# czbiohub-sf/yogo

Measured on AMD Instinct MI355X. Metric: training images/sec (772x1032 gray), higher is better.
Workload: dtype bf16; 1 GPU; BASELINE configs[2]: full train step (fwd+loss+bwd+clamp+AdamW), base_model, 772x1032x1 uint8, 7 classes; per_gpu_batch=128, global_batch=128, parallelism=dp1

## Files before the change

include/yogo_hip.h:

```cpp
#ifndef YOGO_HIP_H
#define YOGO_HIP_H

#include <stddef.h>

#ifdef __cplusplus
extern "C" {
#endif

typedef void* yogo_stream_t;

const char* yogo_hip_last_error(void);
int yogo_hip_abi_version(void);
int yogo_hip_launch_log(int enable);
int yogo_hip_launch_log_read(char* buf, size_t cap, size_t* needed);


int yogo_conv_packed_bytes(int Cin, int Cout, int ksize, int stride, int mode, size_t* bytes);
int yogo_conv_pack_f32(const float* w_oihw, float* packed, int Cin, int Cout, int ksize, int stride, int mode,
                       yogo_stream_t stream);
int yogo_conv2d_fwd_stats_shape(int B, int Cin, int Cout, int IH, int IW, int ksize, int stride, int* rows, int* mpad);
int yogo_conv2d_fwd_f32(const float* in, const float* packed, const float* bias, float* out, float* out_pre,
                        const float* chan_scale, float* stats_part, int B, int Cin, int Cout, int IH, int IW, int ksize,
                        int stride, int act, yogo_stream_t stream);
int yogo_conv2d_dgrad_f32(const float* dy, const float* packed_dgrad, float* dx, const float* act_ref, int ref_act,
                          const float* chan_scale, int B, int Cin, int Cout, int IH, int IW, int ksize, int stride,
                          yogo_stream_t stream);
int yogo_conv2d_wgrad_workspace_bytes(int B, int Cin, int Cout, int IH, int IW, int ksize, int stride, size_t* bytes);
int yogo_conv2d_wgrad_f32(const float* x, const float* g, float* dw, float* db, void* workspace, int B, int Cin, int Cout,
                          int IH, int IW, int ksize, int stride, float clip, yogo_stream_t stream);

int yogo_conv_first_stats_rows(int B, int IH, int IW, int stride, int* rows);
int yogo_conv_first_fwd(const void* in, int in_dtype, const float* w_oihw, const float* bias, float* out, float* out_pre,
                        const float* chan_scale, float* stats_part, int B, int Cin, int Cout, int IH, int IW, int stride,
                        int act, yogo_stream_t stream);
int yogo_conv_first_wgrad_rows(int B, int IH, int IW, int stride, int* rows);
int yogo_conv_first_wgrad(const void* in, int in_dtype, const float* dy, float* part, int B, int Cin, int Cout, int IH,
                          int IW, int stride, yogo_stream_t stream);

int yogo_bn_finalize(const float* part, int rows, int row_stride, int C, long long count, float eps, float momentum,
                     float* mean_out, float* invstd_out, float* running_mean, float* running_var,
                     long long* num_batches_tracked, yogo_stream_t stream);
int yogo_bn_apply_act(const float* z, float* y, const float* mean, const float* invstd_or_var, int stat_is_var, float eps,
                      const float* gamma, const float* beta, int B, int C, int HW, int act, yogo_stream_t stream);
int yogo_bn_invstd(const float* var, float eps, float* invstd, int C, yogo_stream_t stream);
int yogo_bn_bwd_rows(int B, int HW, int* rows);
int yogo_bn_bwd(const float* g, const float* z, float* dz, const float* mean, const float* invstd, const float* gamma,
                const float* beta, int act, float* dgamma, float* dbeta, float* part, float* sums, int B, int C, int HW,
                int training, float clip, yogo_stream_t stream);
int yogo_partials_reduce(float* part, int rows, int N, float clip, float* out, yogo_stream_t stream);
int yogo_channel_sum(const float* g, int B, int C, int HW, float clip, float* out, yogo_stream_t stream);

int yogo_decode_fwd(const float* raw, float* out, const float* cxs, const float* cys, int B, int P, int Sy, int Sx,
                    float anchor_w, float anchor_h, float width_multiplier, float height_multiplier, int inference,
                    yogo_stream_t stream);
int yogo_decode_bwd(const float* raw, const float* out, const float* gout, float* graw, int B, int P, int Sy, int Sx,
                    int inference, yogo_stream_t stream);

int yogo_decode_bwd_bf16(const float* raw, const float* out, const float* gout, void* graw8c, int B, int P, int Sy, int Sx,
                         int inference, yogo_stream_t stream);

int yogo_loss_workspace_bytes(int B, int Sy, int Sx, size_t* bytes);
int yogo_loss_fwd_bwd(const float* pred, const float* label, float* grad, float* loss_out, void* workspace, int B, int P,
                      int Sy, int Sx, float no_obj_weight, float iou_weight, float classify_weight, float label_smoothing,
                      yogo_stream_t stream);

int yogo_decode_loss_bwd_bf16(const float* raw, const float* label, const float* cxs, const float* cys, void* graw8c, float* loss_out,
                              void* workspace, int B, int P, int Sy, int Sx, float anchor_w, float anchor_h, float width_multiplier,
                              float height_multiplier, float no_obj_weight, float iou_weight, float classify_weight,
                              float label_smoothing, yogo_stream_t stream);

int yogo_format_preds_workspace_bytes(int B, int Sy, int Sx, size_t* bytes);
int yogo_format_preds_batched(const float* pred, float* out_rows, long long* out_cells, int* out_count, void* workspace,
                              int B, int P, int Sy, int Sx, int cap, double obj_thresh, double iou_thresh, int box_format,
                              double min_class_confidence_threshold, yogo_stream_t stream);
int yogo_decode_format_preds_batched(const float* raw, const float* cxs, const float* cys, float* out_rows, long long* out_cells,
                                     int* out_count, void* workspace, int B, int P, int Sy, int Sx, int cap, float anchor_w,
                                     float anchor_h, float width_multiplier, float height_multiplier, int inference,
                                     double obj_thresh, double iou_thresh, int box_format, double min_class_confidence_threshold,
                                     yogo_stream_t stream);
int yogo_head1x1_decode_fwd_bf16(const void* x, const void* packed, const float* bias, float* out, const float* cxs, const float* cys,
                                 int B, int Cin, int P, int Sy, int Sx, float anchor_w, float anchor_h, float width_multiplier,
                                 float height_multiplier, int inference, yogo_stream_t stream);

int yogo_match_workspace_bytes(int B, int Sy, int Sx, int cap, size_t* bytes);
int yogo_match_preds_labels_batched(const float* rows, const int* counts, const float* labels, int* meta, int* pair_label,
                                    int* pair_pred, int* un_label, int* un_pred, float* lab_out, void* workspace, int B, int P, int Sy,
                                    int Sx, int cap, yogo_stream_t stream);
int yogo_match_gather(const float* rows, const float* lab_out, const int* meta, const int* pair_label, const int* pair_pred,
                      const int* un_label, const int* un_pred, float* preds, float* labels, float* missed, float* extra, int B, int P,
                      int cap, long long K, long long Km, long long Ke, yogo_stream_t stream);
int yogo_metrics_state_layout(int C, int T, int nbins, long long* offsets);
int yogo_metrics_accumulate(const float* rows, const float* lab_out, const int* meta, const int* pair_label, const int* pair_pred,
                            const int* un_label, const int* un_pred, const double* roc_thresholds, int T, const double* cal_edges,
                            int nbins, long long* acc, double* bin_conf, double* partial, float* map_rows, long long map_cap, int B,
                            int P, int cap, yogo_stream_t stream);

int yogo_pred_sink_state_layout(int C, long long* offsets);
int yogo_pred_sink_workspace_bytes(int B, size_t* bytes);
int yogo_pred_sink_append(const float* rows, const int* counts, int B, int cap, int P, int mode, int count_classes,
                          long long first_img_id, int img_h, int img_w, long long* state, float* arena, long long arena_cap,
                          int* img_counts, long long img_cap, void* workspace, yogo_stream_t stream);

int yogo_bf16_channel_blocks(int C);
int yogo_conv_bf16_packed_bytes(int Cin, int Cout, int ksize, int mode, size_t* bytes);
int yogo_conv_bf16_pack(const float* w_oihw, const float* scale, void* packed, int Cin, int Cout, int ksize, int mode,
                        yogo_stream_t stream);
int yogo_conv2d_fwd_bf16_stats_shape(int B, int Cin, int Cout, int IH, int IW, int ksize, int stride, int* rows, int* mpad);
int yogo_conv2d_fwd_bf16(const void* in, const void* packed, const float* bias, void* out, float* out_f32,
                         const float* chan_scale, float* stats_part, int B, int Cin, int Cout, int IH, int IW, int ksize,
                         int stride, int act, yogo_stream_t stream);
int yogo_conv2d_fwd_bf16_pre(const void* in, const void* packed, const float* bias, void* out, void* out_pre,
                             const float* chan_scale, int B, int Cin, int Cout, int IH, int IW, int ksize, int stride, int act,
                             yogo_stream_t stream);
int yogo_conv_bf16_pack_blocks(int Cin, int Cout, int ksize, int mode, int* blocks);
int yogo_conv_bf16_pack_multi(const void* table, int n, int total_blocks, yogo_stream_t stream);
int yogo_bf16_signs_bytes(int B, int C, int H, int W, size_t* bytes);
int yogo_conv2d_fwd_bf16_signs(const void* in, const void* packed, const float* bias, void* out, void* signs,
                               const float* chan_scale, int B, int Cin, int Cout, int IH, int IW, int ksize, int stride, int act,
                               yogo_stream_t stream);
int yogo_conv2d_dgrad_bf16_signs(const void* dy, const void* packed_dgrad, void* dx, const void* signs,
                                 const float* chan_scale, int B, int Cin, int Cout, int IH, int IW, int ksize, int stride,
                                 yogo_stream_t stream);
int yogo_conv2d_dgrad_bf16(const void* dy, const void* packed_dgrad, void* dx, const void* act_ref, int ref_act,
                           const float* chan_scale, int B, int Cin, int Cout, int IH, int IW, int ksize, int stride,
                           yogo_stream_t stream);
int yogo_conv2d_wgrad_bf16in(const void* x, const void* g, float* dw, float* db, void* workspace, int B, int Cin, int Cout,
                             int IH, int IW, int ksize, int stride, float clip, yogo_stream_t stream);
int yogo_conv2d_wgrad_bf16_workspace_bytes(int B, int Cin, int Cout, int IH, int IW, int ksize, int stride, size_t* bytes);
int yogo_conv2d_wgrad_bf16(const void* x, const void* g, float* dw, float* db, void* workspace, int B, int Cin, int Cout,
                           int IH, int IW, int ksize, int stride, float clip, yogo_stream_t stream);
int yogo_wgrad_reduce_queue_create(void** queue_out);
int yogo_wgrad_reduce_queue_destroy(void* queue);
int yogo_wgrad_reduce_queue_reset(void* queue);
int yogo_wgrad_reduce_flush(void* queue, yogo_stream_t stream);
int yogo_conv2d_wgrad_bf16_deferred(const void* x, const void* g, float* dw, float* db, void* workspace, int B, int Cin, int Cout, int IH,
                                    int IW, int ks, int stride, float clip, void* queue, yogo_stream_t stream);
int yogo_conv_first_fwd_bf16(const void* in, int in_dtype, const float* w, const float* bias, void* out, int B, int Cin,
                             int Cout, int IH, int IW, int stride, int act, yogo_stream_t stream);
int yogo_conv_first_fwd_train_bf16(const void* in, int in_dtype, const float* w, const float* bias, void* out_bf16,
                                   const float* chan_scale, float* stats_part, int B, int Cin, int Cout, int IH, int IW,
                                   int stride, int act, yogo_stream_t stream);
int yogo_conv_first_wgrad_bf16g(const void* in, int in_dtype, const void* dy_bf16, float* part, int B, int Cin, int Cout,
                                int IH, int IW, int stride, yogo_stream_t stream);
int yogo_conv_first_bn_wgrad_cols(int Cin, int Cout, int* cols);
int yogo_conv_first_bn_wgrad_bf16(const void* in, int in_dtype, const void* g, const void* z, const float* mean,
                                  const float* invstd, const float* gamma, const float* beta, float* part, int B, int Cin,
                                  int Cout, int IH, int IW, int stride, int act, yogo_stream_t stream);
int yogo_conv_first_bn_wgrad_finalize(const float* sums, const float* mean, const float* invstd, const float* gamma,
                                      const float* w_oihw, float* dw, float* dgamma, float* dbeta, int B, int Cin, int Cout,
                                      int IH, int IW, int stride, int training, float clip, yogo_stream_t stream);
int yogo_bn_apply_act_bf16(const void* z, void* y, const float* mean, const float* invstd_or_var, int stat_is_var, float eps,
                           const float* gamma, const float* beta, int B, int C, int HW, int act, yogo_stream_t stream);
int yogo_bn_bwd_bf16_rows(int B, int HW, int* rows);
int yogo_bn_stats_bf16(const void* z, float* part, int B, int C, int HW, yogo_stream_t stream);
int yogo_bn_bwd_bf16(const void* g, const void* z, void* dz, const float* mean, const float* invstd, const float* gamma,
                     const float* beta, int act, float* dgamma, float* dbeta, float* part, float* sums, int B, int C, int HW,
                     int training, float clip, yogo_stream_t stream);
int yogo_bn_bwd_bf16_head(const void* gh, const float* head_w, int P, const void* z, void* dz, const float* mean, const float* invstd,
                          const float* gamma, const float* beta, int act, float* dgamma, float* dbeta, float* part, float* sums, int B,
                          int C, int HW, int training, float clip, yogo_stream_t stream);
int yogo_nchw_f32_to_bf16_8c(const float* in, void* out, int B, int C, int HW, yogo_stream_t stream);
int yogo_bf16_8c_to_nchw_f32(const void* in, float* out, int B, int C, int HW, yogo_stream_t stream);

int yogo_conv_first_mfma_supported(int in_dtype, int Cin, int Cout, int IH, int IW, int stride);
int yogo_conv_first_mfma_stats_rows(int B, int IH, int IW, int* rows);
int yogo_conv_first_mfma(const void* in, const float* w, const float* bias, void* z, void* y, const float* mean,
                         const float* invstd, const float* gamma, const float* beta, float* stats_part, int B, int Cout, int IH,
                         int IW, int act, yogo_stream_t stream);

int yogo_conv_first_gram_rows(int B, int IH, int IW, int* rows);
int yogo_conv_first_gram(const void* in, void* part, double* gram, float* gram_f32, int B, int IH, int IW, yogo_stream_t stream);
int yogo_bn_stats_from_gram(const double* gram, const float* w, const float* bias, int Cout, long long count, float eps,
                            float momentum, float* mean_out, float* invstd_out, float* running_mean, float* running_var,
                            long long* num_batches_tracked, yogo_stream_t stream);
int yogo_conv_first_bn_wgrad_bf16_xg(const void* in, int in_dtype, const void* g, const void* z, const float* mean,
                                     const float* invstd, const float* gamma, const float* beta, float* part, int B, int Cin,
                                     int Cout, int IH, int IW, int stride, int act, yogo_stream_t stream);
int yogo_conv_first_bn_wgrad_finalize_xg(const float* sums, const float* gram, const float* mean, const float* invstd,
                                         const float* gamma, const float* w_oihw, float* dw, float* dgamma, float* dbeta, int B,
                                         int Cin, int Cout, int IH, int IW, int stride, int training, float clip,
                                         yogo_stream_t stream);
int yogo_conv_first_mfma_signs(const void* in, const float* w, const float* bias, void* z, void* y, void* signs, const float* mean,
                               const float* invstd, const float* gamma, const float* beta, int B, int Cout, int IH, int IW, int act,
                               yogo_stream_t stream);
int yogo_conv_first_bn_wgrad_xs_supported(int in_dtype, int Cin, int Cout, int IH, int IW, int stride, int act);
int yogo_conv_first_bn_wgrad_bf16_xs(const void* in, int in_dtype, const void* g, const void* signs, const float* mean,
                                     const float* invstd, const float* gamma, const float* beta, float* part, int B, int Cin,
                                     int Cout, int IH, int IW, int stride, int act, yogo_stream_t stream);
int yogo_conv_first_bn_wgrad_finalize_xs(const float* sums, const float* gram, const float* mean, const float* invstd,
                                         const float* gamma, const float* w_oihw, float* dw, float* dgamma, float* dbeta, int B,
                                         int Cin, int Cout, int IH, int IW, int stride, int training, float clip,
                                         yogo_stream_t stream);
int yogo_conv2d_dgrad_first_bwd_supported(int Cmid, int Cout1, int H, int W, int B, int act0);
int yogo_conv2d_dgrad_first_bwd_rows(int B, int H, int W, int with_wgrad, int* rows);
int yogo_conv2d_dgrad_bf16_first_bwd(const void* g, const void* packed, const void* image, const void* signs, float* part, int B, int Cmid,
                                     int Cout1, int H, int W, int act0, yogo_stream_t stream);
int yogo_conv2d_dgrad_wgrad_first_bwd_workspace_bytes(int B, int H, int W, size_t* bytes);
int yogo_conv2d_dgrad_wgrad_bf16_first_bwd(const void* g, const void* packed, const void* x, const void* image, const void* signs, float* part,
                                           float* dw, float* db, void* workspace, int B, int Cmid, int Cout1, int H, int W, int act0,
                                           float clip, void* queue, yogo_stream_t stream);

int yogo_comm_unique_id_bytes(void);
int yogo_comm_unique_id(void* id_out_host);
int yogo_comm_init(int rank, int world, const void* unique_id_host, void** comm_out);
int yogo_comm_allreduce_flat(void* comm, float* buf, size_t count, yogo_stream_t stream);
int yogo_comm_broadcast_flat(void* comm, void* buf, size_t bytes, int root, yogo_stream_t stream);
int yogo_comm_destroy(void* comm);

int yogo_labels_rasterize(const float* labels, const int* offsets, float* out, int* status, int B, int Sx, int Sy,
                          int box_format, yogo_stream_t stream);
int yogo_flip_batch(const void* img_in, void* img_out, int elem_bytes, const float* lab_in, float* lab_out, int B, int C, int H,
                    int W, int Sy, int Sx, int hflip, int vflip, yogo_stream_t stream);

int yogo_blobgen_max_n(int* n);
int yogo_blobgen_place(const int* table, int num_thumbnails, const int* indices, int S, int n, int H, int W, long long seed,
                       long long epoch, int* boxes, float* rows, int* counts, int* background, yogo_stream_t stream);
int yogo_blobgen_compose(const unsigned char* atlas, long long atlas_bytes, const int* table, const int* boxes, const int* counts,
                         const int* background, const int* positions, int S, int n, int H, int W, void* out, int elem_bytes,
                         yogo_stream_t stream);
int yogo_blobgen_label_rows(const float* rows, const int* counts, int S, int n, float* flat, int* offsets, yogo_stream_t stream);

int yogo_image_cache_gather(const unsigned char* cache, int S, const int* slots, int B, int C, int H, int W, void* out, int out_fp32,
                            yogo_stream_t stream);

int yogo_zarr_unpack(const unsigned char* staged, long long staged_bytes, const long long* tile_off, const int* tile_k, int B, int gh,
                     int gw, int ch, int cw, int cn, int order_f, int fill, int H, int W, int top, int left, int OH, int OW, void* out,
                     int out_fp32, yogo_stream_t stream);

int yogo_adamw_step(float* p, const float* g, float* m, float* v, long long n, int step, double lr, double beta1,
                    double beta2, double eps, double weight_decay, double grad_scale, yogo_stream_t stream);

#ifdef __cplusplus
}
#endif
#endif
```

yogo_amd/csrc/bn.hip:

```cpp
#include "common.h"

__global__ __launch_bounds__(256) void bn_finalize_kernel(const float* __restrict__ part, int rows, int row_stride, int C,
                                                          double count, float eps, float momentum,
                                                          float* __restrict__ mean_out, float* __restrict__ invstd_out,
                                                          float* __restrict__ running_mean, float* __restrict__ running_var,
                                                          long long* __restrict__ num_batches_tracked) {
  __shared__ double sh[2][32][8];
  const int cl = threadIdx.x & 7, slice = threadIdx.x >> 3;
  const int c = blockIdx.x * 8 + cl;
  double s = 0.0, q = 0.0;
  if (c < C) {
    int r = slice;
    for (; r + 7 * 32 < rows; r += 8 * 32) {
      float2 v[8];
#pragma unroll
      for (int j = 0; j < 8; ++j) v[j] = *reinterpret_cast<const float2*>(part + ((size_t)(r + j * 32) * row_stride + c) * 2);
#pragma unroll
      for (int j = 0; j < 8; ++j) {
        s += (double)v[j].x;
        q += (double)v[j].y;
      }
    }
    for (; r < rows; r += 32) {
      const float2 v = *reinterpret_cast<const float2*>(part + ((size_t)r * row_stride + c) * 2);
// ... 211 lines not shown
                       gamma, beta, C, HW, act);
  } else {
    dim3 grid(plane_blocks(HW, 4), B * C);
    hipLaunchKernelGGL((bn_apply_act_kernel<false>), grid, dim3(256), 0, stream, z, y, mean, invstd_or_var, stat_is_var, eps,
                       gamma, beta, C, HW, act);
  }
  YOGO_CHECK_LAUNCH("bn_apply_act");
  return YOGO_OK;
}

extern "C" int yogo_bn_invstd(const float* var, float eps, float* invstd, int C, hipStream_t stream) {
  YOGO_CHECK_ARG(var && invstd && C > 0, "bn_invstd: bad arguments");
  hipLaunchKernelGGL(bn_invstd_kernel, dim3(cdiv(C, 256)), dim3(256), 0, stream, var, eps, invstd, C);
  YOGO_CHECK_LAUNCH("bn_invstd");
  return YOGO_OK;
}

extern "C" int yogo_bn_bwd_rows(int B, int HW, int* rows) {
  YOGO_CHECK_ARG(rows != nullptr, "bn_bwd_rows: null");
  *rows = B * plane_blocks(HW, 8);
  return YOGO_OK;
}

extern "C" int yogo_bn_bwd(const float* g, const float* z, float* dz, const float* mean, const float* invstd,
                           const float* gamma, const float* beta, int act, float* dgamma, float* dbeta, float* part,
                           float* sums, int B, int C, int HW, int training, float clip, hipStream_t stream) {
  YOGO_CHECK_ARG(g && z && dz && mean && invstd && gamma && beta && dgamma && dbeta && part && sums, "bn_bwd: null pointer");
  YOGO_CHECK_ARG(B > 0 && C > 0 && HW > 0, "bn_bwd: bad shape");
  const int nb = plane_blocks(HW, 8);
  hipLaunchKernelGGL(bn_bwd_reduce_kernel, dim3(nb, B * C), dim3(256), 0, stream, g, z, mean, invstd, gamma, beta, act, part, C, HW);
  hipLaunchKernelGGL(bn_bwd_finalize_kernel, dim3(C), dim3(256), 0, stream, part, B * nb, C, clip, dgamma, dbeta, sums, sums + C);
  hipLaunchKernelGGL(bn_bwd_apply_kernel, dim3(nb, B * C), dim3(256), 0, stream, g, z, dz, mean, invstd, gamma, beta, act, sums,
                     sums + C, 1.0f / ((float)B * (float)HW), training, C, HW);
  YOGO_CHECK_LAUNCH("bn_bwd");
  return YOGO_OK;
}

__global__ __launch_bounds__(256) void partials_fold_kernel(float* __restrict__ part, int rows, int N, int S) {
  const int j = blockIdx.x * 256 + threadIdx.x;
  const int s = blockIdx.y;
  if (j >= N) return;
  double acc = 0.0;
  int r = s;
  for (; r + 7 * S < rows; r += 8 * S) {
    float v8[8];
#pragma unroll
    for (int k = 0; k < 8; ++k) v8[k] = part[(size_t)(r + k * S) * N + j];
#pragma unroll
    for (int k = 0; k < 8; ++k) acc += (double)v8[k];
  }
  for (; r < rows; r += S) acc += (double)part[(size_t)r * N + j];
  part[(size_t)s * N + j] = (float)acc;
}

extern "C" int yogo_partials_reduce(float* part, int rows, int N, float clip, float* out, hipStream_t stream) {
  YOGO_CHECK_ARG(part && out && rows > 0 && N > 0, "partials_reduce: bad arguments");
  if (rows > 64) {
    const int S = 64;
    hipLaunchKernelGGL(partials_fold_kernel, dim3(cdiv(N, 256), S), dim3(256), 0, stream, part, rows, N, S);
    rows = S;
  }
  hipLaunchKernelGGL(partials_reduce_kernel, dim3(cdiv(N, 256)), dim3(256), 0, stream, part, rows, N, clip, out);
  YOGO_CHECK_LAUNCH("partials_reduce");
  return YOGO_OK;
}

extern "C" int yogo_channel_sum(const float* g, int B, int C, int HW, float clip, float* out, hipStream_t stream) {
  YOGO_CHECK_ARG(g && out && B > 0 && C > 0 && HW > 0, "channel_sum: bad arguments");
  hipLaunchKernelGGL(channel_sum_kernel, dim3(C), dim3(256), 0, stream, g, B, C, HW, clip, out);
  YOGO_CHECK_LAUNCH("channel_sum");
  return YOGO_OK;
}

typedef __bf16 bf16x8_t __attribute__((ext_vector_type(8)));
typedef unsigned int u32x4_t __attribute__((ext_vector_type(4)));

struct Bn8cParams {
  float mu[8], sc[8], sh[8], ga[8], is[8];
};

__device__ __forceinline__ void bn8c_load(Bn8cParams& q, int cb, int C, const float* mean, const float* invstd_or_var,
                                          int stat_is_var, float eps, const float* gamma, const float* beta) {
#pragma unroll
  for (int j = 0; j < 8; ++j) {
    const int c = min(cb * 8 + j, C - 1);
    const float is = stat_is_var ? 1.0f / sqrtf(invstd_or_var[c] + eps) : invstd_or_var[c];
    q.mu[j] = mean[c];
    q.is[j] = is;
    q.ga[j] = gamma[c];
    q.sc[j] = is * gamma[c];
    q.sh[j] = beta[c];
  }
}

__global__ __launch_bounds__(256) void bn_apply_act_8c_kernel(const u32x4_t* __restrict__ z, u32x4_t* __restrict__ y,
                                                              const float* __restrict__ mean,
                                                              const float* __restrict__ invstd_or_var, int stat_is_var, float eps,
                                                              const float* __restrict__ gamma, const float* __restrict__ beta,
                                                              int C, int Cb, int HW, int act) {
  const int plane = blockIdx.y;
  const int cb = plane % Cb;
  Bn8cParams q;
  bn8c_load(q, cb, C, mean, invstd_or_var, stat_is_var, eps, gamma, beta);
  const u32x4_t* zp = z + (size_t)plane * HW;
  u32x4_t* yp = y + (size_t)plane * HW;
  float sh2[8];
#pragma unroll
  for (int j = 0; j < 8; ++j) sh2[j] = fmaf(-q.mu[j], q.sc[j], q.sh[j]);
  for (int i = blockIdx.x * 256 + threadIdx.x; i < HW; i += gridDim.x * 256) {
    const bf16x8_t v = __builtin_bit_cast(bf16x8_t, zp[i]);
    bf16x8_t o;
#pragma unroll
    for (int j = 0; j < 8; ++j) {
      const float r = act_fwd(fmaf((float)v[j], q.sc[j], sh2[j]), act);
      o[j] = (cb * 8 + j < C) ? (__bf16)r : (__bf16)0.f;
    }
    yp[i] = __builtin_bit_cast(u32x4_t, o);
  }
}

__global__ __launch_bounds__(256) void bn_stats_8c_kernel(const u32x4_t* __restrict__ z, float* __restrict__ part, int C, int Cb,
                                                          int HW) {
  __shared__ float sh[4][16];
  const int plane = blockIdx.y;
  const int cb = plane % Cb, b = plane / Cb;
  const u32x4_t* zp = z + (size_t)plane * HW;
  float s[8], t[8];
#pragma unroll
  for (int j = 0; j < 8; ++j) s[j] = t[j] = 0.f;
  for (int i = blockIdx.x * 256 + threadIdx.x; i < HW; i += gridDim.x * 256) {
    const bf16x8_t zv = __builtin_bit_cast(bf16x8_t, zp[i]);
#pragma unroll
    for (int j = 0; j < 8; ++j) {
      const float v = (float)zv[j];
      s[j] += v;
      t[j] = fmaf(v, v, t[j]);
    }
  }
  const int lane = threadIdx.x & 63, wave = threadIdx.x >> 6;
#pragma unroll
  for (int j = 0; j < 8; ++j) {
    const float a = wave_sum(s[j]), c = wave_sum(t[j]);
    if (lane == 0) {
      sh[wave][2 * j] = a;
      sh[wave][2 * j + 1] = c;
    }
  }
  __syncthreads();
  if (threadIdx.x < 16) {
    const int j = threadIdx.x >> 1;
    if (cb * 8 + j < C)
      part[((size_t)(b * gridDim.x + blockIdx.x) * C + cb * 8 + j) * 2 + (threadIdx.x & 1)] =
          sh[0][threadIdx.x] + sh[1][threadIdx.x] + sh[2][threadIdx.x] + sh[3][threadIdx.x];
  }
}

__global__ __launch_bounds__(256) void bn_bwd_reduce_8c_kernel(const u32x4_t* __restrict__ g, const u32x4_t* __restrict__ z,
                                                               const float* __restrict__ mean, const float* __restrict__ invstd,
                                                               const float* __restrict__ gamma, const float* __restrict__ beta,
                                                               int act, float* __restrict__ part, int C, int Cb, int HW) {
  __shared__ float sh[4][16];
  const int plane = blockIdx.y;
  const int cb = plane % Cb, b = plane / Cb;
  Bn8cParams q;
  bn8c_load(q, cb, C, mean, invstd, 0, 0.f, gamma, beta);
  const u32x4_t* gp = g + (size_t)plane * HW;
  const u32x4_t* zp = z + (size_t)plane * HW;
  float s[8], t[8];
#pragma unroll
  for (int j = 0; j < 8; ++j) s[j] = t[j] = 0.f;
  for (int i = blockIdx.x * 256 + threadIdx.x; i < HW; i += gridDim.x * 256) {
    const bf16x8_t gv = __builtin_bit_cast(bf16x8_t, gp[i]);
    const bf16x8_t zv = __builtin_bit_cast(bf16x8_t, zp[i]);
#pragma unroll
    for (int j = 0; j < 8; ++j) {
      const float xh = ((float)zv[j] - q.mu[j]) * q.is[j];
      const float ge = (float)gv[j] * act_bwd_factor(fmaf(xh, q.ga[j], q.sh[j]), act);
      s[j] += ge;
      t[j] += ge * xh;
    }
  }
  const int lane = threadIdx.x & 63, wave = threadIdx.x >> 6;
#pragma unroll
  for (int j = 0; j < 8; ++j) {
    const float a = wave_sum(s[j]), c = wave_sum(t[j]);
    if (lane == 0) {
      sh[wave][2 * j] = a;
      sh[wave][2 * j + 1] = c;
    }
  }
  __syncthreads();
  if (threadIdx.x < 16) {
    const int j = threadIdx.x >> 1;
    if (cb * 8 + j < C)
      part[((size_t)(b * gridDim.x + blockIdx.x) * C + cb * 8 + j) * 2 + (threadIdx.x & 1)] =
          sh[0][threadIdx.x] + sh[1][threadIdx.x] + sh[2][threadIdx.x] + sh[3][threadIdx.x];
  }
}

__global__ __launch_bounds__(256) void bn_bwd_apply_8c_kernel(const u32x4_t* __restrict__ g, const u32x4_t* __restrict__ z,
                                                              u32x4_t* __restrict__ dz, const float* __restrict__ mean,
                                                              const float* __restrict__ invstd, const float* __restrict__ gamma,
                                                              const float* __restrict__ beta, int act,
                                                              const float* __restrict__ sum_g, const float* __restrict__ sum_gx,
                                                              float inv_count, int training, int C, int Cb, int HW) {
  const int plane = blockIdx.y;
  const int cb = plane % Cb;
  Bn8cParams q;
  bn8c_load(q, cb, C, mean, invstd, 0, 0.f, gamma, beta);
  float mg[8], mgx[8];
#pragma unroll
  for (int j = 0; j < 8; ++j) {
    const int c = min(cb * 8 + j, C - 1);
    mg[j] = training ? sum_g[c] * inv_count : 0.f;
    mgx[j] = training ? sum_gx[c] * inv_count : 0.f;
  }
  const u32x4_t* gp = g + (size_t)plane * HW;
  const u32x4_t* zp = z + (size_t)plane * HW;
  u32x4_t* dp = dz + (size_t)plane * HW;
  for (int i = blockIdx.x * 256 + threadIdx.x; i < HW; i += gridDim.x * 256) {
    const bf16x8_t gv = __builtin_bit_cast(bf16x8_t, gp[i]);
    const bf16x8_t zv = __builtin_bit_cast(bf16x8_t, zp[i]);
    bf16x8_t o;
#pragma unroll
    for (int j = 0; j < 8; ++j) {
      const float xh = ((float)zv[j] - q.mu[j]) * q.is[j];
      const float ge = (float)gv[j] * act_bwd_factor(fmaf(xh, q.ga[j], q.sh[j]), act);
      const float r = q.sc[j] * (ge - mg[j] - xh * mgx[j]);
      o[j] = (cb * 8 + j < C) ? (__bf16)r : (__bf16)0.f;
    }
    dp[i] = __builtin_bit_cast(u32x4_t, o);
  }
}

__global__ __launch_bounds__(256) void nchw_f32_to_8c_kernel(const float* __restrict__ in, u32x4_t* __restrict__ out, int C, int Cb,
                                                             int HW) {
  const int plane = blockIdx.y;
  const int cb = plane % Cb, b = plane / Cb;
  for (int i = blockIdx.x * 256 + threadIdx.x; i < HW; i += gridDim.x * 256) {
    bf16x8_t o;
#pragma unroll
    for (int j = 0; j < 8; ++j) {
      const int c = cb * 8 + j;
      o[j] = (c < C) ? (__bf16)in[((size_t)b * C + c) * HW + i] : (__bf16)0.f;
    }
    out[(size_t)plane * HW + i] = __builtin_bit_cast(u32x4_t, o);
  }
}

__global__ __launch_bounds__(256) void nchw8c_to_f32_kernel(const u32x4_t* __restrict__ in, float* __restrict__ out, int C, int Cb,
                                                            int HW) {
  const int plane = blockIdx.y;
  const int cb = plane % Cb, b = plane / Cb;
  for (int i = blockIdx.x * 256 + threadIdx.x; i < HW; i += gridDim.x * 256) {
    const bf16x8_t v = __builtin_bit_cast(bf16x8_t, in[(size_t)plane * HW + i]);
#pragma unroll
    for (int j = 0; j < 8; ++j) {
      const int c = cb * 8 + j;
      if (c < C) out[((size_t)b * C + c) * HW + i] = (float)v[j];
    }
  }
}

static inline int cb_of(int C) { return ((C + 15) / 16) * 2; }

extern "C" int yogo_bn_apply_act_bf16(const void* z, void* y, const float* mean, const float* invstd_or_var, int stat_is_var,
                                      float eps, const float* gamma, const float* beta, int B, int C, int HW, int act,
                                      hipStream_t stream) {
  YOGO_CHECK_ARG(z && y && mean && invstd_or_var && gamma && beta && C > 0 && HW > 0 && B >= 0, "bn_apply_act_bf16: bad arguments");
  if (B == 0) return YOGO_OK;
  const int Cb = cb_of(C);
  YOGO_CHECK_ARG(B * Cb <= 65535, "bn_apply_act_bf16: batch * channel blocks exceeds 65535");
  hipLaunchKernelGGL(bn_apply_act_8c_kernel, dim3(plane_blocks(HW, 4), B * Cb), dim3(256), 0, stream,
                     reinterpret_cast<const u32x4_t*>(z), reinterpret_cast<u32x4_t*>(y), mean, invstd_or_var, stat_is_var, eps,
                     gamma, beta, C, Cb, HW, act);
  YOGO_CHECK_LAUNCH("bn_apply_act_bf16");
  return YOGO_OK;
}

extern "C" int yogo_bn_bwd_bf16_rows(int B, int HW, int* rows) {
  YOGO_CHECK_ARG(rows != nullptr, "bn_bwd_bf16_rows: null");
  *rows = B * plane_blocks(HW, 4);
  return YOGO_OK;
}

extern "C" int yogo_bn_bwd_bf16(const void* g, const void* z, void* dz, const float* mean, const float* invstd,
                                const float* gamma, const float* beta, int act, float* dgamma, float* dbeta, float* part,
                                float* sums, int B, int C, int HW, int training, float clip, hipStream_t stream) {
  YOGO_CHECK_ARG(g && z && dz && mean && invstd && gamma && beta && dgamma && dbeta && part && sums, "bn_bwd_bf16: null pointer");
  YOGO_CHECK_ARG(B > 0 && C > 0 && HW > 0, "bn_bwd_bf16: bad shape");
  const int Cb = cb_of(C), nb = plane_blocks(HW, 4);
  YOGO_CHECK_ARG(B * Cb <= 65535, "bn_bwd_bf16: batch * channel blocks exceeds 65535");
  const u32x4_t* g4 = reinterpret_cast<const u32x4_t*>(g);
  const u32x4_t* z4 = reinterpret_cast<const u32x4_t*>(z);
  hipLaunchKernelGGL(bn_bwd_reduce_8c_kernel, dim3(nb, B * Cb), dim3(256), 0, stream, g4, z4, mean, invstd, gamma, beta, act, part, C,
                     Cb, HW);
  hipLaunchKernelGGL(bn_bwd_finalize_kernel, dim3(C), dim3(256), 0, stream, part, B * nb, C, clip, dgamma, dbeta, sums, sums + C);
  hipLaunchKernelGGL(bn_bwd_apply_8c_kernel, dim3(nb, B * Cb), dim3(256), 0, stream, g4, z4, reinterpret_cast<u32x4_t*>(dz), mean,
                     invstd, gamma, beta, act, sums, sums + C, 1.0f / ((float)B * (float)HW), training, C, Cb, HW);
  YOGO_CHECK_LAUNCH("bn_bwd_bf16");
  return YOGO_OK;
}

typedef float f32x4_t __attribute__((ext_vector_type(4)));
typedef unsigned int u32x2_t __attribute__((ext_vector_type(2)));
typedef __bf16 bf16x4_t __attribute__((ext_vector_type(4)));
struct BnHeadLane {
  bf16x8_t wop;
  float mu[4], is[4], ga[4], sh[4], sc[4];
};
__device__ __forceinline__ void bn_head_lane(BnHeadLane& L, const float* __restrict__ hw, int P, int C, int cp, int c16, int g4, const float* mean,
                                             const float* invstd, const float* gamma, const float* beta) {
#pragma unroll
  for (int j = 0; j < 8; ++j) {
    const int k = 8 * g4 + j;
    L.wop[j] = (k < P) ? (__bf16)hw[(size_t)k * C + 16 * cp + c16] : (__bf16)0.f;
  }
#pragma unroll
  for (int i = 0; i < 4; ++i) {
    const int c = 16 * cp + 4 * g4 + i;
    L.mu[i] = mean[c]; L.is[i] = invstd[c]; L.ga[i] = gamma[c]; L.sh[i] = beta[c]; L.sc[i] = invstd[c] * gamma[c];
  }
}
__device__ __forceinline__ void bn_head_fetch(const BnHeadLane& L, const u32x4_t* __restrict__ ghp, const u32x2_t* __restrict__ zp2, int HW, int px, int g4,
                                              float (&gb)[4], float (&zf)[4]) {
  const bool valid = px < HW;
  u32x4_t gop = {0u, 0u, 0u, 0u};
  if (valid && g4 < 2) gop = ghp[(size_t)g4 * HW + px];
  u32x2_t zr = {0u, 0u};
  if (valid) zr = zp2[(size_t)px * 2];
  const f32x4_t d = __builtin_amdgcn_mfma_f32_16x16x32_bf16(L.wop, __builtin_bit_cast(bf16x8_t, gop), f32x4_t{0.f, 0.f, 0.f, 0.f}, 0, 0, 0);
  const bf16x4_t zv = __builtin_bit_cast(bf16x4_t, zr);
#pragma unroll
  for (int i = 0; i < 4; ++i) {
    gb[i] = (float)(__bf16)d[i];
    zf[i] = (float)zv[i];
  }
}
__global__ __launch_bounds__(256) void bn_bwd_reduce_head_kernel(const u32x4_t* __restrict__ gh, const float* __restrict__ hw, int P,
                                                                 const u32x4_t* __restrict__ z, const float* __restrict__ mean,
                                                                 const float* __restrict__ invstd, const float* __restrict__ gamma,
                                                                 const float* __restrict__ beta, int act, float* __restrict__ part, int C, int Cb, int HW) {
  __shared__ float sh[4][32];
  const int cp = blockIdx.y % (Cb / 2), b = blockIdx.y / (Cb / 2);
  const int lane = threadIdx.x & 63, wave = threadIdx.x >> 6, c16 = lane & 15, g4 = lane >> 4;
  BnHeadLane L;
  bn_head_lane(L, hw, P, C, cp, c16, g4, mean, invstd, gamma, beta);
  const u32x4_t* ghp = gh + (size_t)b * 2 * HW;
  const u32x2_t* zp2 = reinterpret_cast<const u32x2_t*>(z + ((size_t)b * Cb + 2 * cp + (g4 >> 1)) * HW) + (g4 & 1);
  float s[4] = {0.f, 0.f, 0.f, 0.f}, t[4] = {0.f, 0.f, 0.f, 0.f};
  for (int px0 = (blockIdx.x * 4 + wave) * 16; px0 < HW; px0 += gridDim.x * 64) {
    float gb[4], zf[4];
    bn_head_fetch(L, ghp, zp2, HW, px0 + c16, g4, gb, zf);
#pragma unroll
    for (int i = 0; i < 4; ++i) {
      const float xh = (zf[i] - L.mu[i]) * L.is[i];
      const float ge = gb[i] * act_bwd_factor(fmaf(xh, L.ga[i], L.sh[i]), act);
      s[i] += ge;
      t[i] += ge * xh;
    }
  }
#pragma unroll
  for (int i = 0; i < 4; ++i) {
    float a = s[i], c = t[i];
#pragma unroll
    for (int o = 8; o > 0; o >>= 1) {
      a += __shfl_xor(a, o, 64);
      c += __shfl_xor(c, o, 64);
    }
    if (c16 == 0) {
      sh[wave][2 * (4 * g4 + i)] = a;
      sh[wave][2 * (4 * g4 + i) + 1] = c;
    }
  }
  __syncthreads();
  if (threadIdx.x < 32)
    part[((size_t)(b * gridDim.x + blockIdx.x) * C + 16 * cp + (threadIdx.x >> 1)) * 2 + (threadIdx.x & 1)] =
        sh[0][threadIdx.x] + sh[1][threadIdx.x] + sh[2][threadIdx.x] + sh[3][threadIdx.x];
}
__global__ __launch_bounds__(256) void bn_bwd_apply_head_kernel(const u32x4_t* __restrict__ gh, const float* __restrict__ hw, int P,
                                                                const u32x4_t* __restrict__ z, u32x4_t* __restrict__ dz, const float* __restrict__ mean,
                                                                const float* __restrict__ invstd, const float* __restrict__ gamma,
                                                                const float* __restrict__ beta, int act, const float* __restrict__ sum_g,
                                                                const float* __restrict__ sum_gx, float inv_count, int training, int C, int Cb, int HW) {
  const int cp = blockIdx.y % (Cb / 2), b = blockIdx.y / (Cb / 2);
  const int lane = threadIdx.x & 63, wave = threadIdx.x >> 6, c16 = lane & 15, g4 = lane >> 4;
  BnHeadLane L;
  bn_head_lane(L, hw, P, C, cp, c16, g4, mean, invstd, gamma, beta);
  float mg[4], mgx[4];
#pragma unroll
  for (int i = 0; i < 4; ++i) {
    const int c = 16 * cp + 4 * g4 + i;
    mg[i] = training ? sum_g[c] * inv_count : 0.f;
    mgx[i] = training ? sum_gx[c] * inv_count : 0.f;
  }
  const u32x4_t* ghp = gh + (size_t)b * 2 * HW;
  const size_t plane_u = ((size_t)b * Cb + 2 * cp + (g4 >> 1)) * HW;
  const u32x2_t* zp2 = reinterpret_cast<const u32x2_t*>(z + plane_u) + (g4 & 1);
  u32x2_t* dp2 = reinterpret_cast<u32x2_t*>(dz + plane_u) + (g4 & 1);
  for (int px0 = (blockIdx.x * 4 + wave) * 16; px0 < HW; px0 += gridDim.x * 64) {
    const int px = px0 + c16;
    float gb[4], zf[4];
    bn_head_fetch(L, ghp, zp2, HW, px, g4, gb, zf);
    bf16x4_t o;
#pragma unroll
    for (int i = 0; i < 4; ++i) {
      const float xh = (zf[i] - L.mu[i]) * L.is[i];
      const float ge = gb[i] * act_bwd_factor(fmaf(xh, L.ga[i], L.sh[i]), act);
      o[i] = (__bf16)(L.sc[i] * (ge - mg[i] - xh * mgx[i]));
    }
    if (px < HW) dp2[(size_t)px * 2] = __builtin_bit_cast(u32x2_t, o);
  }
}
extern "C" int yogo_bn_bwd_bf16_head(const void* gh, const float* head_w, int P, const void* z, void* dz, const float* mean, const float* invstd,
                                     const float* gamma, const float* beta, int act, float* dgamma, float* dbeta, float* part, float* sums,
                                     int B, int C, int HW, int training, float clip, hipStream_t stream) {
  YOGO_CHECK_ARG(gh && head_w && z && dz && mean && invstd && gamma && beta && dgamma && dbeta && part && sums, "bn_bwd_bf16_head: null pointer");
  YOGO_CHECK_ARG(B > 0 && C > 0 && (C % 16) == 0 && HW > 0 && P > 0 && P <= 16, "bn_bwd_bf16_head: bad shape");
  const int Cb = cb_of(C), nb = plane_blocks(HW, 4);
  YOGO_CHECK_ARG(B * Cb <= 65535, "bn_bwd_bf16_head: batch * channel blocks exceeds 65535");
  const u32x4_t* g4 = reinterpret_cast<const u32x4_t*>(gh);
  const u32x4_t* z4 = reinterpret_cast<const u32x4_t*>(z);
  if (yogo_launch_log_enabled()) {
    yogo_launch_log("bn_bwd_reduce_head_kernel | B=%d C=%d HW=%d P=%d act=%d grid=%dx%d", B, C, HW, P, act, nb, B * (Cb / 2));
    yogo_launch_log("bn_bwd_apply_head_kernel | B=%d C=%d HW=%d P=%d act=%d training=%d grid=%dx%d", B, C, HW, P, act, training, nb, B * (Cb / 2));
  }
  hipLaunchKernelGGL(bn_bwd_reduce_head_kernel, dim3(nb, B * (Cb / 2)), dim3(256), 0, stream, g4, head_w, P, z4, mean, invstd, gamma, beta, act, part, C, Cb,
                     HW);
  hipLaunchKernelGGL(bn_bwd_finalize_kernel, dim3(C), dim3(256), 0, stream, part, B * nb, C, clip, dgamma, dbeta, sums, sums + C);
  hipLaunchKernelGGL(bn_bwd_apply_head_kernel, dim3(nb, B * (Cb / 2)), dim3(256), 0, stream, g4, head_w, P, z4, reinterpret_cast<u32x4_t*>(dz), mean, invstd,
                     gamma, beta, act, sums, sums + C, 1.0f / ((float)B * (float)HW), training, C, Cb, HW);
  YOGO_CHECK_LAUNCH("bn_bwd_bf16_head");
  return YOGO_OK;
}

extern "C" int yogo_bn_stats_bf16(const void* z, float* part, int B, int C, int HW, hipStream_t stream) {
  YOGO_CHECK_ARG(z && part && B > 0 && C > 0 && HW > 0, "bn_stats_bf16: bad arguments");
  const int Cb = cb_of(C), nb = plane_blocks(HW, 4);
  YOGO_CHECK_ARG(B * Cb <= 65535, "bn_stats_bf16: batch * channel blocks exceeds 65535");
  hipLaunchKernelGGL(bn_stats_8c_kernel, dim3(nb, B * Cb), dim3(256), 0, stream, reinterpret_cast<const u32x4_t*>(z), part, C, Cb, HW);
  YOGO_CHECK_LAUNCH("bn_stats_bf16");
  return YOGO_OK;
}

extern "C" int yogo_nchw_f32_to_bf16_8c(const float* in, void* out, int B, int C, int HW, hipStream_t stream) {
  YOGO_CHECK_ARG(in && out && B > 0 && C > 0 && HW > 0, "nchw_f32_to_bf16_8c: bad arguments");
  const int Cb = cb_of(C);
  hipLaunchKernelGGL(nchw_f32_to_8c_kernel, dim3(plane_blocks(HW, 2), B * Cb), dim3(256), 0, stream, in,
                     reinterpret_cast<u32x4_t*>(out), C, Cb, HW);
  YOGO_CHECK_LAUNCH("nchw_f32_to_bf16_8c");
  return YOGO_OK;
}

extern "C" int yogo_bf16_8c_to_nchw_f32(const void* in, float* out, int B, int C, int HW, hipStream_t stream) {
  YOGO_CHECK_ARG(in && out && B > 0 && C > 0 && HW > 0, "bf16_8c_to_nchw_f32: bad arguments");
  const int Cb = cb_of(C);
  hipLaunchKernelGGL(nchw8c_to_f32_kernel, dim3(plane_blocks(HW, 2), B * Cb), dim3(256), 0, stream,
                     reinterpret_cast<const u32x4_t*>(in), out, C, Cb, HW);
  YOGO_CHECK_LAUNCH("bf16_8c_to_nchw_f32");
  return YOGO_OK;
}
```

yogo_amd/csrc/conv_bf16.hip:

```cpp
#include "common.h"
#include "conv_bf16_ws.h"
#include "conv_bf16_ws16.h"
#include "conv_bf16_ws3.h"
#include <type_traits>
#include <utility>
#include <cstdlib>
#include <vector>

typedef float f32x16 __attribute__((ext_vector_type(16)));
typedef __bf16 bf16x8 __attribute__((ext_vector_type(8)));
typedef __bf16 bf16x4 __attribute__((ext_vector_type(4)));
typedef unsigned int u32x4 __attribute__((ext_vector_type(4)));
typedef unsigned int u32x2 __attribute__((ext_vector_type(2)));
typedef int i32x16 __attribute__((ext_vector_type(16)));

#define BF_MAX_TAPS 9
#define BF_LDS_BUDGET (80 * 1024)
#define BF_LDS_MAX (160 * 1024)

struct ConvBf16Params {
  const u32x4* in;
  const u32x4* wp;
  const float* bias;
  u32x2* out;
// ... 1180 lines not shown
  g_diag_stamps = reinterpret_cast<unsigned long long*>(stamps); g_diag_stamps_bytes = stamps_bytes;
  return YOGO_OK;
}
#endif

namespace {

template <int MW, int NW, int NWV, bool S2D, int PF, bool F32, int REF, bool PP, bool LEPI = false>
void bf_launch_one(dim3 grid, int lds_bytes, hipStream_t stream, const ConvBf16Params& p, const char* plan_txt) {
  static bool attr_set = false;
  if (!attr_set) {
    (void)hipFuncSetAttribute(reinterpret_cast<const void*>(&conv_bf16_kernel<MW, NW, NWV, S2D, PF, F32, REF, PP, LEPI>),
                              hipFuncAttributeMaxDynamicSharedMemorySize, BF_LDS_MAX);
    attr_set = true;
  }
  hipLaunchKernelGGL((conv_bf16_kernel<MW, NW, NWV, S2D, PF, F32, REF, PP, LEPI>), grid, dim3(64 * NWV), lds_bytes, stream, p);
  yogo_launch_log("conv_bf16_kernel<%d, %d, %d, %s, %d, %s, %d, %s, %s> | %s", MW, NW, NWV, S2D ? "true" : "false", PF, F32 ? "true" : "false", REF,
                  PP ? "true" : "false", LEPI ? "true" : "false", plan_txt);
}
template <int MW, int NW, int NWV, bool S2D, int PF, bool F32, int REF>
void bf_launch_t(dim3 grid, int lds_bytes, hipStream_t stream, const ConvBf16Params& p, bool use_pp, const char* plan_txt) {
  if constexpr (NWV == 8 && !S2D && !F32) {
    if (use_pp) {
      bf_launch_one<MW, NW, NWV, S2D, PF, F32, REF, true>(grid, lds_bytes, stream, p, plan_txt);
      return;
    }
  }
  if constexpr (NWV == 4 && !S2D && !F32) {
    if (p.lean4) {
      const bool general = p.stats_part != nullptr || p.act == ACT_SILU || p.out_pre != nullptr || ((REF == 1 || REF == 2) && p.ref_act != ACT_LEAKY);
#ifndef BF_NO_LEPI
      if constexpr (REF != 1) {
        if (!general) {
          bf_launch_one<MW, NW, NWV, S2D, PF, F32, REF, true, true>(grid, lds_bytes, stream, p, plan_txt);
          return;
        }
      }
#else
      (void)general;
#endif
      bf_launch_one<MW, NW, NWV, S2D, PF, F32, REF, true>(grid, lds_bytes, stream, p, plan_txt);
      return;
    }
  }
  if constexpr (NWV == 4 && S2D && !F32 && REF != 1) {
    const bool general = p.stats_part != nullptr || p.act == ACT_SILU || p.out_pre != nullptr || (REF == 2 && p.ref_act != ACT_LEAKY);
    if (!general) {
      bf_launch_one<MW, NW, NWV, S2D, PF, F32, REF, false, true>(grid, lds_bytes, stream, p, plan_txt);
      return;
    }
  }
  bf_launch_one<MW, NW, NWV, S2D, PF, F32, REF, false>(grid, lds_bytes, stream, p, plan_txt);
}

int launch_conv_bf16(const void* in, const void* packed, const float* bias, void* out, float* out_f32, void* out_pre, const void* act_ref,
                     int ref_act, void* signs, bool signs_read, const float* chan_scale, float* stats_part, int B, int K, int M, int IH, int IW, int OH,
                     int OW, int ks, int a, int s2d, int act, hipStream_t stream, int* stats_rows, int* stats_mpad) {
  const int T = ks * ks, pad = ks == 3 ? 1 : 0;
  if (in != nullptr && g_bf_ws && !s2d && a == 1 && ks == 3 && out_f32 == nullptr && out_pre == nullptr && act_ref == nullptr && !signs_read &&
      stats_part == nullptr && (act == ACT_NONE || act == ACT_LEAKY) && !(signs != nullptr && act != ACT_LEAKY) &&
      conv_bf16_ws_eligible(K, M, IH, IW, B)) {
    ConvWsParams q{};
    q.in = in; q.wp = packed; q.bias = bias; q.out = out; q.signs = reinterpret_cast<unsigned char*>(signs); q.chan_scale = chan_scale;
    q.B = B; q.Kb = bf_kb_of(K); q.IH = IH; q.IW = IW; q.act = act;
#ifdef YOGO_DIAG
    q.dbg = g_diag_dbg;
    q.stamps = (g_diag_stamps != nullptr && g_diag_stamps_bytes >= 512 * 128) ? g_diag_stamps : nullptr;
    if (q.stamps) (void)hipMemsetAsync(g_diag_stamps, 0, 512 * 128, stream);
#endif
    if (conv_bf16_ws_plan(&q)) {
      if ((g_bf_ws16 == 2 || (g_bf_ws16 == 1 && bias == nullptr)) && act == ACT_NONE && signs == nullptr && chan_scale == nullptr &&
          conv_bf16_ws16_eligible(K, M, IH, IW, B))
        return launch_conv_bf16_ws16(q, stream);
      return launch_conv_bf16_ws(q, stream);
    }
  }
  if (in != nullptr && g_bf_ws && !s2d && a == 2 && ks == 3 && out_f32 == nullptr && out_pre == nullptr && act_ref == nullptr && !signs_read &&
      stats_part == nullptr && (act == ACT_NONE || act == ACT_LEAKY) && !(signs != nullptr && act != ACT_LEAKY) && conv_bf16_ws3_eligible(K, M, IH, IW, B)) {
    ConvWs3Params q{};
    q.in = in; q.wp = packed; q.bias = bias; q.out = out; q.signs = reinterpret_cast<unsigned char*>(signs); q.chan_scale = chan_scale;
    q.B = B; q.Kb = bf_kb_of(K); q.IH = IH; q.IW = IW; q.OH = OH; q.OW = OW; q.act = act;
#ifdef YOGO_DIAG
    q.dbg = g_diag_dbg;
    q.stamps = (g_diag_stamps != nullptr && g_diag_stamps_bytes >= 512 * 128) ? g_diag_stamps : nullptr;
    if (q.stamps) (void)hipMemsetAsync(g_diag_stamps, 0, 512 * 128, stream);
#endif
    if (conv_bf16_ws3_plan(&q)) return launch_conv_bf16_ws3(q, stream);
  }
  if (in != nullptr && g_bf_head && ks == 1 && a == 1 && !s2d && out_pre == nullptr && act_ref == nullptr && stats_part == nullptr && act == ACT_NONE &&
      out_f32 != nullptr && out == nullptr && signs == nullptr && chan_scale == nullptr && conv_bf16_head_fwd_eligible(K, M, OH * OW, B))
    return launch_conv_bf16_head_fwd(in, packed, bias, out_f32, B, K, M, OH * OW, stream);
  if (in != nullptr && g_bf_staged && !s2d && ks == 3 && out_f32 == nullptr && out_pre == nullptr && act_ref == nullptr && !signs_read && stats_part == nullptr &&
      (act == ACT_NONE || act == ACT_LEAKY) && !(signs != nullptr && act != ACT_LEAKY) && conv_bf16_staged_eligible(K, M, a, IH, IW, OH, OW, B))
    return launch_conv_bf16_staged(in, packed, bias, out, signs, chan_scale, B, K, M, IH, IW, OH, OW, a, act, stream);
  if (in != nullptr && g_bf_direct && s2d && ks == 3 && out_f32 == nullptr && out_pre == nullptr && act_ref == nullptr && bias == nullptr &&
      stats_part == nullptr && act == ACT_NONE && (!signs_read || (signs != nullptr && ref_act == ACT_LEAKY)) && (signs_read || signs == nullptr) &&
      conv_bf16_s2d_direct_eligible(K, M, OH, OW, B))
    return launch_conv_bf16_s2d_direct(in, packed, out, signs_read ? signs : nullptr, chan_scale, B, K, M, IH, IW, OH, OW, stream);
  const int MW = bf_pick_mw(M);
  const bool small_n = s2d || a == 2;
  const bool wide64 = MW == 2 && !small_n && K >= 64 && OH * OW >= 4096;
  const int NW = MW == 1 ? (small_n ? 2 : 4) : (small_n ? 1 : (wide64 ? 4 : 2));
  const int NWV = (MW == 4 || wide64) ? 8 : 4;
  const int PF = NWV == 8 ? 10 : 16;
  const int Kb = bf_kb_of(K), Mpad = bf_mpad_of(M);
  const int OHt = s2d ? (OH + 1) / 2 : OH, OWt = s2d ? (OW + 1) / 2 : OW;
  BfTiling tl;
  bool planned = false;
  if (NWV == 4) {
    const int ladder[3] = {40 * 1024, 53 * 1024, BF_LDS_BUDGET};
    for (int i = 0; i < 3 && !planned; ++i)
      planned = bf_plan(OHt, OWt, s2d ? 1 : a, s2d ? 6 : T, s2d ? 2 : ks, Kb, MW, NW, NWV, PF, ladder[i], &tl) && tl.dma;
  }
  bool ring = false;
  if (s2d && MW == 4 && Kb >= 8 && g_bf_ring) {
    ring = bf_plan(OHt, OWt, 1, 6, 2, Kb, MW, NW, NWV, 5, BF_LDS_MAX, &tl, false, 2, 4, 2);
    planned = ring;
  }
  if (!planned) planned = bf_plan(OHt, OWt, s2d ? 1 : a, s2d ? 6 : T, s2d ? 2 : ks, Kb, MW, NW, NWV, PF, BF_LDS_MAX, &tl);
  if (!planned) {
    yogo_set_error("conv_bf16: no LDS tiling fits (K=%d M=%d OW=%d a=%d)", K, M, OW, a);
    return YOGO_ERR_ARG;
  }
  int rowdma = 0, lwp = 0;
  if (!s2d && NWV == 4 && T == 9 && tl.CKb == 2 && tl.dma == 2 && out_f32 == nullptr && g_bf_lean4 && g_bf_rowdma) {
    const int ladder[3] = {40 * 1024, 53 * 1024, BF_LDS_BUDGET};
    int level = 0;
    while (level < 2 && tl.lds_bytes > ladder[level]) ++level;
    BfTiling tr;
    if (tl.lds_bytes <= ladder[level] && bf_plan_rows(OHt, OWt, a, T, ks, Kb, MW, NW, NWV, ladder[level], &tr, &lwp)) {
      tl = tr;
      rowdma = 1;
    }
  }
  dim3 grid(tl.ncb * tl.tiles_per_band, (Mpad / (32 * MW)) * (s2d ? 2 : 1), B);
  if (stats_rows) *stats_rows = B * (int)grid.x;
  if (stats_mpad) *stats_mpad = Mpad;
  if (in == nullptr) return YOGO_OK;
  ConvBf16Params p{};
  p.in = reinterpret_cast<const u32x4*>(in); p.wp = reinterpret_cast<const u32x4*>(packed); p.bias = bias;
  p.out = reinterpret_cast<u32x2*>(out); p.out_f32 = out_f32; p.out_pre = reinterpret_cast<u32x2*>(out_pre);
  p.act_ref = reinterpret_cast<const u32x2*>(act_ref); p.ref_act = ref_act; p.signs = reinterpret_cast<unsigned char*>(signs); p.chan_scale = chan_scale; p.stats_part = stats_part;
  p.B = B; p.Kb = Kb; p.M = M; p.Mpad = Mpad; p.Mb = bf_kb_of(M);
  p.IH = IH; p.IW = IW; p.OH = OH; p.OW = OW; p.T = T;
  if (s2d) {
    p.a = 1; p.dy_min = 0; p.dx_min = 0; p.span_y = 2; p.span_x = 2;
  } else {
    p.a = a; p.dy_min = -pad; p.dx_min = -pad; p.span_y = ks; p.span_x = ks;
  }
  p.ncb = tl.ncb; p.TW = tl.TW; p.tiles_per_band = tl.tiles_per_band;
  {
    auto magic = [](int d) -> unsigned { return d <= 1 ? 0xFFFFFFFFu : (unsigned)(((1ull << 32) + (unsigned)d - 1ull) / (unsigned)d); };
    const int a_ = s2d ? 1 : a, span_ = s2d ? 2 : ks;
    const int bw_last = OWt - (tl.ncb - 1) * tl.TW;
    p.m_gx = magic((int)grid.x); p.m_gy = magic((int)grid.y); p.m_gxy = magic((int)(grid.x * grid.y)); p.m_tpb = magic(tl.tiles_per_band);
    p.m_bw = magic(tl.TW); p.m_bwl = magic(bw_last);
    p.m_lw = magic((tl.TW - 1) * a_ + span_); p.m_lwl = magic((bw_last - 1) * a_ + span_);
  }
  p.CKb = tl.CKb; p.ckb_shift = tl.CKb == 8 ? 3 : (tl.CKb == 4 ? 2 : 1); p.nchunk = Kb / tl.CKb;
  p.ldsw_off = tl.ldsw_off; p.lds_dummy = tl.lds_dummy; p.act = act;
  p.dma = tl.dma; p.ni_slots = tl.ni_slots; p.n_slots = tl.n_slots; p.bufu = tl.bufu; p.bufs = tl.dma == 1 ? tl.bufu : 0;
  p.ring = ring ? 1 : 0;
  p.lean4 = (!s2d && NWV == 4 && T == 9 && tl.CKb == 2 && tl.dma == 2 && out_f32 == nullptr && g_bf_lean4) ? 1 : 0;
  p.rowdma = rowdma; p.lwp = lwp;
#ifdef YOGO_DIAG
  p.dbg = g_diag_dbg;
  if (g_diag_nodma && (tl.lds_dummy + 1) * 16 <= BF_LDS_MAX) p.dma = 0;
  {
    const size_t nwg = (size_t)grid.x * grid.y * grid.z;
    if (g_diag_stamps != nullptr && nwg * 128 <= g_diag_stamps_bytes) {
      (void)hipMemsetAsync(g_diag_stamps, 0, nwg * 128, stream);
      p.stamps = g_diag_stamps;
    }
  }
#endif
  if ((act_ref != nullptr || signs_read) && bias != nullptr) {
    yogo_set_error("conv_bf16: an activation reference goes with a data gradient (no bias)");
    return YOGO_ERR_ARG;
  }
  if (B == 0) return YOGO_OK;
  int lds_bytes = max(p.dma ? tl.lds_bytes : (tl.lds_dummy + 1) * 16, (2 + 2 * NWV) * 32 * MW * 4);
  const bool use_pp = NWV == 8 && !s2d && T == 9 && p.dma == 1 && tl.CKb == 2 && tl.ni_slots <= 5 && tl.n_slots - tl.ni_slots <= 5 && g_bf_pp;
  if (use_pp) {
    p.ni_slots = 5; p.n_slots = 10; p.ldsw_off = 5 * 64 * NWV; p.bufu = 10 * 64 * NWV; p.bufs = p.bufu;
    lds_bytes = 2 * p.bufu * 16;
  }
  char plan_txt[256] = "";
  if (yogo_launch_log_enabled())
    snprintf(plan_txt, sizeof(plan_txt), "K=%d M=%d in=%dx%d out=%dx%d a=%d s2d=%d T=%d ncb=%d TW=%d tiles_per_band=%d CKb=%d nchunk=%d rows=%d LW=%d lds=%d dma=%d slots=%d+%d rowpitch=%d grid=%ux%ux%u",
             K, M, IH, IW, OH, OW, a, s2d, T, tl.ncb, tl.TW, tl.tiles_per_band, tl.CKb, Kb / tl.CKb, tl.rows_max, tl.LW, lds_bytes, p.dma, tl.ni_slots,
             tl.n_slots - tl.ni_slots, rowdma ? lwp : 0, grid.x, grid.y, grid.z);
#define BFLAUNCH__(MW_, NW_, NWV_, S2D_, PF_, F32_, REF_)                                                               \
  bf_launch_t<MW_, NW_, NWV_, S2D_, PF_, F32_, REF_>(grid, lds_bytes, stream, p, use_pp, plan_txt)
#define BFLAUNCH_(MW_, NW_, NWV_, S2D_, PF_, F32_)                             \
  do {                                                                         \
    if (act_ref != nullptr) BFLAUNCH__(MW_, NW_, NWV_, S2D_, PF_, false, 1);   \
    else if (signs_read) BFLAUNCH__(MW_, NW_, NWV_, S2D_, PF_, false, 2);      \
    else if (signs != nullptr && NWV_ != 8) BFLAUNCH__(MW_, NW_, NWV_, S2D_, PF_, false, 3); \
    else BFLAUNCH__(MW_, NW_, NWV_, S2D_, PF_, F32_, 0);                       \
  } while (0)
#define BFLAUNCH(MW_, NW_, NWV_, S2D_, PF_)                                    \
  do {                                                                         \
    if (out_f32 != nullptr) BFLAUNCH_(MW_, NW_, NWV_, S2D_, PF_, true);        \
    else BFLAUNCH_(MW_, NW_, NWV_, S2D_, PF_, false);                          \
  } while (0)
  if (s2d) {
    if (MW == 4) BFLAUNCH_(4, 1, 8, true, 10, false);
    else if (MW == 2) BFLAUNCH_(2, 1, 4, true, 16, false);
    else BFLAUNCH_(1, 2, 4, true, 16, false);
  } else if (a == 2) {
    if (MW == 4) BFLAUNCH(4, 1, 8, false, 10);
    else if (MW == 2) BFLAUNCH(2, 1, 4, false, 16);
    else BFLAUNCH(1, 2, 4, false, 16);
  } else {
    if (MW == 4) BFLAUNCH(4, 2, 8, false, 10);
    else if (MW == 2 && wide64) BFLAUNCH(2, 4, 8, false, 10);
    else if (MW == 2) BFLAUNCH(2, 2, 4, false, 16);
    else BFLAUNCH(1, 4, 4, false, 16);
  }
#undef BFLAUNCH
#undef BFLAUNCH_
#undef BFLAUNCH__
  YOGO_CHECK_LAUNCH("conv_bf16");
  return YOGO_OK;
}

int check_bf16_conv(int B, int Cin, int Cout, int IH, int IW, int ks, int stride) {
  YOGO_CHECK_ARG((ks == 3 || ks == 1) && (stride == 1 || stride == 2) && !(ks == 1 && stride != 1) && B >= 0 && Cin > 0 &&
                     Cout > 0 && IH > 0 && IW > 0, "conv_bf16: unsupported shape");
  return YOGO_OK;
}

}

extern "C" int yogo_conv2d_fwd_bf16_stats_shape(int B, int Cin, int Cout, int IH, int IW, int ks, int stride, int* rows, int* mpad) {
  if (int e = check_bf16_conv(B, Cin, Cout, IH, IW, ks, stride)) return e;
  const int pad = ks == 3 ? 1 : 0;
  return launch_conv_bf16(nullptr, nullptr, nullptr, nullptr, nullptr, nullptr, nullptr, 0, nullptr, false, nullptr, nullptr, B, Cin, Cout, IH, IW,
                          (IH + 2 * pad - ks) / stride + 1, (IW + 2 * pad - ks) / stride + 1, ks, stride, 0, 0, nullptr, rows, mpad);
}

extern "C" int yogo_conv2d_fwd_bf16(const void* in, const void* packed, const float* bias, void* out, float* out_f32,
                                    const float* chan_scale, float* stats_part, int B, int Cin, int Cout, int IH, int IW,
                                    int ks, int stride, int act, hipStream_t stream) {
  YOGO_CHECK_ARG(in && packed && (out || out_f32), "conv2d_fwd_bf16: null pointer");
  if (int e = check_bf16_conv(B, Cin, Cout, IH, IW, ks, stride)) return e;
  const int pad = ks == 3 ? 1 : 0;
  return launch_conv_bf16(in, packed, bias, out, out_f32, nullptr, nullptr, 0, nullptr, false, chan_scale, stats_part, B, Cin, Cout, IH, IW,
                          (IH + 2 * pad - ks) / stride + 1, (IW + 2 * pad - ks) / stride + 1, ks, stride, 0, act, stream,
                          nullptr, nullptr);
}

extern "C" int yogo_conv2d_fwd_bf16_pre(const void* in, const void* packed, const float* bias, void* out, void* out_pre,
                                        const float* chan_scale, int B, int Cin, int Cout, int IH, int IW, int ks, int stride,
                                        int act, hipStream_t stream) {
  YOGO_CHECK_ARG(in && packed && out && out_pre, "conv2d_fwd_bf16_pre: null pointer");
  if (int e = check_bf16_conv(B, Cin, Cout, IH, IW, ks, stride)) return e;
  const int pad = ks == 3 ? 1 : 0;
  return launch_conv_bf16(in, packed, bias, out, nullptr, out_pre, nullptr, 0, nullptr, false, chan_scale, nullptr, B, Cin, Cout, IH, IW,
                          (IH + 2 * pad - ks) / stride + 1, (IW + 2 * pad - ks) / stride + 1, ks, stride, 0, act, stream,
                          nullptr, nullptr);
}

extern "C" int yogo_bf16_signs_bytes(int B, int C, int H, int W, size_t* bytes) {
  YOGO_CHECK_ARG(bytes && B >= 0 && C > 0 && H > 0 && W > 0, "bf16_signs_bytes: bad arguments");
  *bytes = (size_t)B * H * W * (bf_mpad_of(C) / 8);
  return YOGO_OK;
}

extern "C" int yogo_conv2d_fwd_bf16_signs(const void* in, const void* packed, const float* bias, void* out, void* signs,
                                          const float* chan_scale, int B, int Cin, int Cout, int IH, int IW, int ks, int stride,
                                          int act, hipStream_t stream) {
  YOGO_CHECK_ARG(in && packed && out && signs, "conv2d_fwd_bf16_signs: null pointer");
  if (int e = check_bf16_conv(B, Cin, Cout, IH, IW, ks, stride)) return e;
  const int pad = ks == 3 ? 1 : 0;
  return launch_conv_bf16(in, packed, bias, out, nullptr, nullptr, nullptr, 0, signs, false, chan_scale, nullptr, B, Cin, Cout, IH, IW,
                          (IH + 2 * pad - ks) / stride + 1, (IW + 2 * pad - ks) / stride + 1, ks, stride, 0, act, stream,
                          nullptr, nullptr);
}

extern "C" int yogo_conv2d_dgrad_bf16_signs(const void* dy, const void* packed_dgrad, void* dx, const void* signs,
                                            const float* chan_scale, int B, int Cin, int Cout, int IH, int IW, int ks, int stride,
                                            hipStream_t stream) {
  YOGO_CHECK_ARG(dy && packed_dgrad && dx && signs, "conv2d_dgrad_bf16_signs: null pointer");
  if (int e = check_bf16_conv(B, Cin, Cout, IH, IW, ks, stride)) return e;
  const int pad = ks == 3 ? 1 : 0;
  const int OHf = (IH + 2 * pad - ks) / stride + 1, OWf = (IW + 2 * pad - ks) / stride + 1;
  return launch_conv_bf16(dy, packed_dgrad, nullptr, dx, nullptr, nullptr, nullptr, ACT_LEAKY, const_cast<void*>(signs), true, chan_scale,
                          nullptr, B, Cout, Cin, OHf, OWf, IH, IW, ks, 1, (stride == 2 && ks == 3) ? 1 : 0, ACT_NONE, stream, nullptr,
                          nullptr);
}

extern "C" int yogo_conv2d_dgrad_bf16(const void* dy, const void* packed_dgrad, void* dx, const void* act_ref, int ref_act,
                                      const float* chan_scale, int B, int Cin, int Cout, int IH, int IW, int ks, int stride,
                                      hipStream_t stream) {
  YOGO_CHECK_ARG(dy && packed_dgrad && dx, "conv2d_dgrad_bf16: null pointer");
  if (int e = check_bf16_conv(B, Cin, Cout, IH, IW, ks, stride)) return e;
  const int pad = ks == 3 ? 1 : 0;
  const int OHf = (IH + 2 * pad - ks) / stride + 1, OWf = (IW + 2 * pad - ks) / stride + 1;
  return launch_conv_bf16(dy, packed_dgrad, nullptr, dx, nullptr, nullptr, act_ref, ref_act, nullptr, false, chan_scale, nullptr, B, Cout, Cin, OHf, OWf,
                          IH, IW, ks, 1, (stride == 2 && ks == 3) ? 1 : 0, ACT_NONE, stream, nullptr, nullptr);
}

extern "C" int yogo_conv_first_fwd_bf16(const void* in, int in_dtype, const float* w, const float* bias, void* out, int B,
                                        int Cin, int Cout, int IH, int IW, int stride, int act, hipStream_t stream) {
  YOGO_CHECK_ARG(in && w && out, "conv_first_fwd_bf16: null pointer");
  YOGO_CHECK_ARG((Cin == 1 || Cin == 3) && Cout > 0 && (stride == 1 || stride == 2) && (in_dtype == 0 || in_dtype == 1) && B >= 0,
                 "conv_first_fwd_bf16: unsupported shape");
  ConvFirstBf16Params p{};
  p.in = in; p.w = w; p.bias = bias; p.out = reinterpret_cast<u32x4*>(out);
  p.B = B; p.Cin = Cin; p.Cout = Cout; p.Mb = bf_kb_of(Cout); p.IH = IH; p.IW = IW; p.stride = stride; p.act = act;
  p.OH = (IH - 1) / stride + 1; p.OW = (IW - 1) / stride + 1;
  if (B == 0) return YOGO_OK;
  dim3 grid(cdiv(p.OH * p.OW, 256), B);
  if (in_dtype == 0 && Cin == 1) hipLaunchKernelGGL((conv_first_bf16_kernel<uint8_t, 1>), grid, dim3(256), 0, stream, p);
  else if (in_dtype == 0) hipLaunchKernelGGL((conv_first_bf16_kernel<uint8_t, 3>), grid, dim3(256), 0, stream, p);
  else if (Cin == 1) hipLaunchKernelGGL((conv_first_bf16_kernel<float, 1>), grid, dim3(256), 0, stream, p);
  else hipLaunchKernelGGL((conv_first_bf16_kernel<float, 3>), grid, dim3(256), 0, stream, p);
  YOGO_CHECK_LAUNCH("conv_first_fwd_bf16");
  return YOGO_OK;
}
```

yogo_amd/csrc/conv_bf16_ws.h:

```cpp
#pragma once
#include "common.h"

#define WS_PT 256
#define WS_NT 256
#define WS_NI 4
#define WS_WB (9 * 2 * 128 * 16)
#define WS_IB (WS_NI * WS_NT * 16)
#define WS_I0 (2 * WS_WB)
#define WS_STG (WS_I0 + 3 * WS_IB)
#define WS_EB (WS_STG + 32768)
#define WS_ES (WS_EB + 512)
#define WS_MB (WS_ES + 1024)
#define WS_MBS (WS_MB + 4096)
#define WS_LDS_BYTES (WS_MBS + 16)

struct ConvWsParams {
  const void* in;
  const void* wp;
  const float* bias;
  void* out;
  unsigned char* signs;
  const float* chan_scale;
  int B, Kb, IH, IW;
  int ncb, TW, tiles_per_band, gx, ntiles;
  unsigned m_gx, m_tpb, m_bw, m_bwl, m_lw, m_lwl;
  int nchunk, act;
#ifdef YOGO_DIAG
  int dbg;
  unsigned long long* stamps;
#endif
};

bool conv_bf16_ws_eligible(int K, int M, int IH, int IW, int B);
bool conv_bf16_ws_plan(ConvWsParams* p, int slots = WS_NI);
int launch_conv_bf16_ws(const ConvWsParams& p, hipStream_t stream);
```

yogo_amd/csrc/conv_bf16_ws16.h:

```cpp
#pragma once
#include "conv_bf16_ws.h"

#define W16_WSLOT (3 * 2 * 2 * 128 * 16)
#define W16_W0 0
#define W16_ISLOT (2 * WS_IB)
#define W16_I0 (2 * W16_WSLOT)
#define W16_STG (W16_I0 + 2 * W16_ISLOT)
#define W16_EB (W16_STG + 32768)
#define W16_MB (W16_EB + 512)
#define W16_MBS (W16_MB + 1024)
#define W16_LDS_BYTES (W16_MBS + 16)

bool conv_bf16_ws16_eligible(int K, int M, int IH, int IW, int B);
int launch_conv_bf16_ws16(const ConvWsParams& p, hipStream_t stream);
```

yogo_amd/csrc/conv_bf16_ws16.hip:

```cpp
#include "conv_bf16_ws16.h"
#ifndef W16_ASM_INC
#define W16_ASM_INC "conv_bf16_ws16_asm.inc"
#endif
#include W16_ASM_INC
#ifndef W16_ABL
#define W16_ABL 0
#endif
#include <mutex>
#include <type_traits>
#include <utility>

typedef unsigned int u32x4 __attribute__((ext_vector_type(4)));
typedef int i32x4 __attribute__((ext_vector_type(4)));

#define W16_CLOBBER \
  "memory", "scc", "s87", "s88", "s89", "s90", "s91", "s92", "s93", "s94", "s95", \
  "v16", "v17", "v18", "v19", "v20", "v21", "v22", "v23", "v24", "v25", "v26", "v27", "v28", "v29", "v30", "v31", "v32", "v33", "v34", "v35", "v36", "v37", "v38", "v39", "v40", "v41", "v42", "v43", "v44", "v45", "v46", "v47", "v48", "v49", "v50", "v51", "v52", "v53", "v54", "v55", "v56", "v57", "v58", "v59", "v60", "v61", "v62", "v63", "v64", "v65", "v66", "v67", "v68", "v69", "v70", "v71", "v72", "v73", "v74", "v75", "v76", "v77", "v78", "v79", "v80", "v81", "v82", "v83", "v84", "v85", "v86", "v87", "v88", "v89", "v90", "v91", "v92", "v93", "v94", "v95", \
  "a0","a1","a2","a3","a4","a5","a6","a7","a8","a9","a10","a11","a12","a13","a14","a15","a16","a17","a18","a19","a20","a21","a22","a23","a24","a25","a26","a27","a28","a29","a30","a31","a32","a33","a34","a35","a36","a37","a38","a39","a40","a41","a42","a43","a44","a45","a46","a47","a48","a49","a50","a51","a52","a53","a54","a55","a56","a57","a58","a59","a60","a61","a62","a63","a64","a65","a66","a67","a68","a69","a70","a71","a72","a73","a74","a75","a76","a77","a78","a79","a80","a81","a82","a83","a84","a85","a86","a87","a88","a89","a90","a91","a92","a93","a94","a95","a96","a97","a98","a99","a100","a101","a102","a103","a104","a105","a106","a107","a108","a109","a110","a111","a112","a113","a114","a115","a116","a117","a118","a119","a120","a121","a122","a123","a124","a125","a126","a127","a128","a129","a130","a131","a132","a133","a134","a135","a136","a137","a138","a139","a140","a141","a142","a143","a144","a145","a146","a147","a148","a149","a150","a151","a152","a153","a154","a155","a156","a157","a158","a159"

namespace {

__device__ __forceinline__ int w16_udivm(int n, unsigned m) { return (int)__umulhi((unsigned)n, m); }
__device__ __forceinline__ int w16_udivm1(int n, int d, unsigned m) { return d == 1 ? n : (int)__umulhi((unsigned)n, m); }
__device__ __forceinline__ int w16_lane() {
  int l;
  asm volatile("v_mbcnt_lo_u32_b32 %0, -1, 0\n\tv_mbcnt_hi_u32_b32 %0, -1, %0" : "=v"(l));
  return l;
}
__device__ __forceinline__ i32x4 w16_rsrc(const void* ptr, unsigned bytes) {
  const unsigned long long a = reinterpret_cast<unsigned long long>(ptr);
  return i32x4{(int)(unsigned)a, (int)((unsigned)(a >> 32) & 0xFFFFu), (int)bytes, 0x00020000};
}
__device__ __forceinline__ void w16_dma4(i32x4 rs, unsigned lds, int v0, int v1, int v2, int v3, unsigned soff) {
  asm volatile(
      "s_mov_b32 m0, %5\n\ts_nop 4\n\tbuffer_load_dwordx4 %0, %4, %6 offen lds\n\t"
      "s_add_u32 m0, m0, 4096\n\ts_nop 0\n\tbuffer_load_dwordx4 %1, %4, %6 offen lds\n\t"
      "s_add_u32 m0, m0, 4096\n\ts_nop 0\n\tbuffer_load_dwordx4 %2, %4, %6 offen lds\n\t"
      "s_add_u32 m0, m0, 4096\n\ts_nop 0\n\tbuffer_load_dwordx4 %3, %4, %6 offen lds"
      ::"v"(v0), "v"(v1), "v"(v2), "v"(v3), "s"(rs), "s"(lds), "s"(soff) : "memory", "scc");
}
__device__ __forceinline__ void w16_dma6(i32x4 rs, unsigned lds, int voff, unsigned soff, unsigned sj, unsigned sk) {
  unsigned so;
#define W16_PJ "s_add_u32 m0, m0, 4096\n\ts_add_u32 %0, %0, %5\n\tbuffer_load_dwordx4 %1, %2, %0 offen lds\n\t"
#define W16_PK "s_add_u32 m0, m0, 4096\n\ts_add_u32 %0, %0, %6\n\tbuffer_load_dwordx4 %1, %2, %0 offen lds\n\t"
  asm volatile("s_mov_b32 m0, %3\n\ts_mov_b32 %0, %4\n\ts_nop 4\n\tbuffer_load_dwordx4 %1, %2, %0 offen lds\n\t" W16_PJ W16_PK W16_PJ W16_PK W16_PJ
               : "=&s"(so)
               : "v"(voff), "s"(rs), "s"(lds), "s"(soff), "s"(sj), "s"(sk)
               : "memory", "scc");
#undef W16_PJ
#undef W16_PK
}
__device__ __forceinline__ void w16_store16(u32x4 data, int voff, i32x4 rs, unsigned soff) {
  asm volatile("s_nop 4\n\tbuffer_store_dwordx4 %0, %1, %2, %3 offen" ::"v"(data), "v"(voff), "s"(rs), "s"(soff) : "memory");
}

}

template <bool BIAS>
__global__ __launch_bounds__(512) __attribute__((amdgpu_waves_per_eu(2, 2), amdgpu_num_vgpr(96))) void conv_bf16_ws16_kernel(const ConvWsParams p) {
  extern __shared__ __attribute__((aligned(16))) u32x4 smem4[];
  constexpr unsigned OOB = 0x80000000u;
  const int tid = threadIdx.x;
  const int wave = __builtin_amdgcn_readfirstlane(tid >> 6);
  const int team = wave >> 2, tw = wave & 3;
  float* ldsf = reinterpret_cast<float*>(smem4);
  unsigned char* lds = reinterpret_cast<unsigned char*>(smem4);

  const int OH = p.IH, OW = p.IW;
  const int plane = OH * OW, plane16 = plane * 16;
  const int npairs = p.nchunk >> 1, nper = 3 * npairs;

  const unsigned NV = (unsigned)p.ntiles, G = gridDim.x, slot = blockIdx.x;
  const unsigned xq = NV >> 3, xr = NV & 7;
  struct TileS { int b, j0, bw, p0, p1, lastband; };
  auto find_tile = [&](unsigned& k, TileS& t) -> bool {
    for (;; ++k) {
      const unsigned lin = slot + k * G;
      if (lin >= NV) return false;
      const unsigned xcd = lin & 7;
      const int widx = (int)((xcd < xr ? xcd * (xq + 1) : xr * (xq + 1) + (xcd - xr) * xq) + (lin >> 3));
      const int b = w16_udivm1(widx, p.gx, p.m_gx);
      const int bx = widx - b * p.gx;
      const int cb = w16_udivm1(bx, p.tiles_per_band, p.m_tpb);
      const int tb = bx - cb * p.tiles_per_band;
      const int j0 = cb * p.TW;
      const int bw = min(p.TW, OW - j0);
      const int NPb = OH * bw;
      const int p0 = tb * WS_PT;
      if (p0 >= NPb) continue;
      t.b = b; t.j0 = j0; t.bw = bw; t.p0 = p0; t.p1 = min(p0 + WS_PT, NPb); t.lastband = cb == p.ncb - 1;
      return true;
    }
  };
  auto pix_geom = [&](const TileS& t, int q, unsigned& pbase, int& vo) {
    const unsigned m_bw = t.lastband ? p.m_bwl : p.m_bw;
    const int bw = t.bw;
    const int i_lo = w16_udivm(t.p0, m_bw);
    const int pp = t.p0 + q;
    const bool pv = pp < t.p1;
    const int pc = pv ? pp : (t.p1 - 1);
    const int i = w16_udivm(pc, m_bw), j = pc - i * bw;
    pbase = (unsigned)((i - i_lo) * (bw + 2) + j) * 16u;
    vo = pv ? (i * OW + t.j0 + j) * 16 : (int)OOB;
  };
  auto tile_pitch = [&](const TileS& t, unsigned& lw16, unsigned& perkb16) {
    const unsigned m_bw = t.lastband ? p.m_bwl : p.m_bw;
    const int i_lo = w16_udivm(t.p0, m_bw), i_hi = w16_udivm(t.p1 - 1, m_bw);
    lw16 = (unsigned)(t.bw + 2) * 16u;
    perkb16 = (unsigned)(i_hi - i_lo + 3) * lw16;
  };

  unsigned k_ord = 0;
  TileS T{};
  if (!find_tile(k_ord, T)) return;

  if (tid < 128) ldsf[W16_EB / 4 + tid] = (BIAS && p.bias != nullptr) ? p.bias[tid] : 0.f;
  __syncthreads();

  if (team == 1) {
    const int lane = w16_lane();
    const int ttid = tw * 64 + lane;
    const int rowb = p.IW * 16, kcb = p.IH * p.IW * 16;
    const unsigned ibytes = (unsigned)p.Kb * kcb, obytes = 16u * plane16, wbytes = 9u * p.Kb * 2048u;
    const unsigned so_i = 2u * kcb;
    const unsigned wstep = (unsigned)p.Kb * 2048u;
    const i32x4 rs_w = w16_rsrc(p.wp, wbytes);
    const int lane16 = lane * 16;
    const int kbw = tw >> 1, colh = tw & 1;
    auto decode_slots = [&](const TileS& t, int (&voff)[WS_NI]) {
      const unsigned m_bw = t.lastband ? p.m_bwl : p.m_bw;
      const int bw = t.bw;
      const int i_lo = w16_udivm(t.p0, m_bw), i_hi = w16_udivm(t.p1 - 1, m_bw);
      const int rows_in = i_hi - i_lo + 3;
      const int iy0 = i_lo - 1, ix0 = t.j0 - 1;
      const int lw = bw + 2;
      const int per_kb = rows_in * lw;
      const unsigned inv_lw = t.lastband ? p.m_lwl : p.m_lw;
      const unsigned inv_perkb = 0xFFFFFFFFu / (unsigned)per_kb + 1u;
      const int skc = w16_udivm(WS_NT, inv_perkb);
      const int srm = WS_NT - skc * per_kb;
      const int sr = w16_udivm(srm, inv_lw);
      const int sx = srm - sr * lw;
      int kc_ = w16_udivm(ttid, inv_perkb);
      const int rm0 = ttid - kc_ * per_kb;
      int r_ = w16_udivm(rm0, inv_lw);
      int x_ = rm0 - r_ * lw;
#pragma unroll
      for (int i = 0; i < WS_NI; ++i) {
        const int iy_ = iy0 + r_, ix_ = ix0 + x_;
        const bool ok = (kc_ < 2) && (iy_ >= 0) && (iy_ < p.IH) && (ix_ >= 0) && (ix_ < p.IW);
        voff[i] = ok ? kc_ * kcb + iy_ * rowb + ix_ * 16 : (int)OOB;
        x_ += sx; r_ += sr; kc_ += skc;
        if (x_ >= lw) { x_ -= lw; ++r_; }
        if (r_ >= rows_in) { r_ -= rows_in; ++kc_; }
      }
    };
    static_assert(WS_NI == 4, "w16_dma4 issues the four input slots");
    auto req_w = [&](int P, int r, int par) {
      const unsigned soff = (unsigned)(((3 * r) * p.Kb + 4 * P + kbw) * 2048 + colh * 1024);
      w16_dma6(rs_w, (unsigned)(W16_W0 + par * W16_WSLOT + kbw * 2048 + colh * 1024), lane16, soff, 4096u, wstep - 4096u);
    };
    auto req_i = [&](i32x4 rs, const int (&voff)[WS_NI], int cn, int ps, int j) {
      w16_dma4(rs, (unsigned)(W16_I0 + ps * W16_ISLOT + j * WS_IB + tw * 64 * 16), voff[0], voff[1], voff[2], voff[3], (unsigned)cn * so_i);
    };
    const unsigned stg_rd = (unsigned)(W16_STG + tw * 8192 + lane * 16);
    u32x4 fifo[8];
    int f_vo = (int)OOB;
    i32x4 f_rs = w16_rsrc(p.out, 0u);
    int f_cb0 = 0;
    auto fifo_fill = [&](int cb0, int vop, i32x4 rs_o) {
#pragma unroll
      for (int u = 0; u < 8; ++u) fifo[u] = *reinterpret_cast<const u32x4*>(lds + stg_rd + u * 1024);
      f_vo = vop; f_rs = rs_o; f_cb0 = cb0;
    };
    auto fifo_store4 = [&](auto h_tag) {
      constexpr int Hh = decltype(h_tag)::value;
      const i32x4 rs = {__builtin_amdgcn_readfirstlane(f_rs.x), __builtin_amdgcn_readfirstlane(f_rs.y), __builtin_amdgcn_readfirstlane(f_rs.z),
                        __builtin_amdgcn_readfirstlane(f_rs.w)};
      const int cb0 = __builtin_amdgcn_readfirstlane(f_cb0);
#pragma unroll
      for (int u = 4 * Hh; u < 4 * Hh + 4; ++u) w16_store16(fifo[u], (W16_ABL & 2) ? (int)OOB : f_vo, rs, (unsigned)(cb0 + u) * (unsigned)plane16);
    };
    using IC0 = std::integral_constant<int, 0>;
    using IC1 = std::integral_constant<int, 1>;

    int voff[WS_NI];
    decode_slots(T, voff);
    unsigned pbase_ = 0, lw16_ = 0, perkb16_ = 0;
    int vo = (int)OOB, vo_prev = (int)OOB;
    pix_geom(T, ttid, pbase_, vo);
    i32x4 rs_in = w16_rsrc(reinterpret_cast<const unsigned char*>(p.in) + (size_t)T.b * ibytes, ibytes);
    i32x4 rs_out = w16_rsrc(reinterpret_cast<unsigned char*>(p.out) + (size_t)T.b * obytes, obytes);
    i32x4 rs_out_prev = w16_rsrc(p.out, 0u);
    req_i(rs_in, voff, 0, 0, 0);
    req_i(rs_in, voff, 1, 0, 1);
    req_w(0, 0, 0);
    asm volatile("s_waitcnt vmcnt(0)" ::: "memory");
    __builtin_amdgcn_s_barrier();
    bool has_next = true;
    TileS Tn{};
    int voff_n[WS_NI] = {(int)OOB, (int)OOB, (int)OOB, (int)OOB}, vo_n = (int)OOB;
    i32x4 rs_in_n = rs_in, rs_out_n = rs_out;
    while (has_next) {
      int P = 0, r = 0;
      for (int c = 0; c < nper; ++c) {
        {
          const int rn = r == 2 ? 0 : r + 1, Pn = r == 2 ? P + 1 : P;
          if ((W16_ABL & 1) && c >= 1) {
          } else if (c + 1 < nper) req_w(Pn, rn, (c + 1) & 1);
          else if (has_next) req_w(0, 0, 0);
        }
        if (c == 0) {
          fifo_fill(0, vo_prev, rs_out_prev);
          asm volatile("s_waitcnt lgkmcnt(0)" ::: "memory");
          if (!(W16_ABL & 4)) __builtin_amdgcn_s_barrier();
        }
        bool req = false;
        if (r < 2 && !(W16_ABL & 8)) {
          if (P + 1 < npairs) {
            req_i(rs_in, voff, 2 * (P + 1) + r, (P + 1) & 1, r);
            req = true;
          } else if (has_next) {
            if (r == 0) {
#pragma unroll
              for (int i = 0; i < WS_NI; ++i) voff[i] = voff_n[i];
              rs_in = rs_in_n;
            }
            req_i(rs_in, voff, r, 0, r);
            req = true;
          }
        }
        if (c == 0) fifo_store4(IC0{});
        else if (c == 1) fifo_store4(IC1{});
        else if (c == 2) { fifo_fill(8, vo_prev, rs_out_prev); fifo_store4(IC0{}); }
        else if (c == 3) fifo_store4(IC1{});
        const bool dr = c < 4;
        if (c == 0) {
          unsigned kn = k_ord + 1;
          has_next = find_tile(kn, Tn);
          k_ord = kn;
          if (has_next) {
            decode_slots(Tn, voff_n);
            pix_geom(Tn, ttid, pbase_, vo_n);
            tile_pitch(Tn, lw16_, perkb16_);
            rs_in_n = w16_rsrc(reinterpret_cast<const unsigned char*>(p.in) + (size_t)Tn.b * ibytes, ibytes);
            rs_out_n = w16_rsrc(reinterpret_cast<unsigned char*>(p.out) + (size_t)Tn.b * obytes, obytes);
          }
        }
        if (c == 1) {
          *reinterpret_cast<unsigned*>(lds + W16_MB + tw * 256 + ((lane & 15) * 4 + (lane >> 4)) * 4) = pbase_;
          if (tw == 0 && lane == 0) *reinterpret_cast<u32x4*>(lds + W16_MBS) = u32x4{has_next ? 1u : 0u, lw16_, perkb16_, 0u};
          asm volatile("s_waitcnt lgkmcnt(0)" ::: "memory");
        }
        if (dr && req) asm volatile("s_waitcnt vmcnt(8)" ::: "memory");
        else if (dr || req) asm volatile("s_waitcnt vmcnt(4)" ::: "memory");
        else asm volatile("s_waitcnt vmcnt(0)" ::: "memory");
        __builtin_amdgcn_s_barrier();
        if (++r == 3) { r = 0; ++P; }
      }
      vo_prev = vo;
      rs_out_prev = rs_out;
      if (has_next) {
        vo = vo_n;
        rs_out = rs_out_n;
      }
    }
    fifo_fill(0, vo_prev, rs_out_prev);
    asm volatile("s_waitcnt lgkmcnt(0)" ::: "memory");
    if (!(W16_ABL & 4)) __builtin_amdgcn_s_barrier();
    fifo_store4(IC0{});
    fifo_store4(IC1{});
    __builtin_amdgcn_s_barrier();
    fifo_fill(8, vo_prev, rs_out_prev);
    fifo_store4(IC0{});
    fifo_store4(IC1{});
    return;
  }

  __builtin_amdgcn_s_setprio(3);
  const int lane = w16_lane(), c16 = lane & 15, g = lane >> 4;
  const unsigned pa_lane = (unsigned)(W16_W0 + (g >> 1) * 4096 + (g & 1) * 2048 + c16 * 16);
  const unsigned stg = (unsigned)(W16_STG + tw * 8192 + (g >> 1) * 1024 + c16 * 16 + (g & 1) * 8);
  const unsigned eb = (unsigned)(W16_EB + g * 16);
  unsigned lw16, perkb16;
  tile_pitch(T, lw16, perkb16);
  unsigned pbl[4];
#pragma unroll
  for (int pb = 0; pb < 4; ++pb) {
    unsigned pbase;
    int vo_unused;
    pix_geom(T, tw * 64 + pb * 16 + c16, pbase, vo_unused);
    pbl[pb] = pbase + (unsigned)(g & 1) * perkb16 + (unsigned)(g >> 1) * (unsigned)WS_IB + (unsigned)W16_I0;
  }
  __builtin_amdgcn_s_barrier();
  const unsigned kmask = (g & 1) ? 0xFFFFFFFFu : 0u, kconst = (unsigned)(g >> 1) * (unsigned)WS_IB + (unsigned)W16_I0;
  const unsigned mba = (unsigned)(W16_MB + tw * 256 + c16 * 16), mbs = (unsigned)W16_MBS;
  const unsigned npp = (unsigned)((nper - 2) >> 1);
  if constexpr (BIAS)
    asm volatile(W16_TXT_ROLEB
                 :
                 : [pa] "v"(pa_lane), [stg] "v"(stg), [eb] "v"(eb), [q0] "v"(pbl[0]), [q1] "v"(pbl[1]), [q2] "v"(pbl[2]), [q3] "v"(pbl[3]), [mba] "v"(mba),
                   [mbs] "v"(mbs), [kmask] "v"(kmask), [kconst] "v"(kconst), [lw16] "s"(lw16), [npp] "s"(npp)
                 : W16_CLOBBER);
  else
    asm volatile(W16_TXT_ROLE
                 :
                 : [pa] "v"(pa_lane), [stg] "v"(stg), [eb] "v"(eb), [q0] "v"(pbl[0]), [q1] "v"(pbl[1]), [q2] "v"(pbl[2]), [q3] "v"(pbl[3]), [mba] "v"(mba),
                   [mbs] "v"(mbs), [kmask] "v"(kmask), [kconst] "v"(kconst), [lw16] "s"(lw16), [npp] "s"(npp)
                 : W16_CLOBBER);
}

bool conv_bf16_ws16_eligible(int K, int M, int IH, int IW, int B) {
  const int Kb = round_up(K, 16) / 8;
  if (!conv_bf16_ws_eligible(K, M, IH, IW, B)) return false;
  return Kb >= 8 && (Kb % 8) == 0;
}

int launch_conv_bf16_ws16(const ConvWsParams& p, hipStream_t stream) {
  static std::mutex mu;
  static int n_cu_of[64] = {0};
  int dev = 0;
  if (hipGetDevice(&dev) != hipSuccess || dev < 0 || dev >= 64) {
    yogo_set_error("conv_bf16_ws16: hipGetDevice failed");
    return YOGO_ERR_HIP;
  }
  int n_cu;
  {
    std::lock_guard<std::mutex> lk(mu);
    if (n_cu_of[dev] == 0) {
      hipError_t e = hipFuncSetAttribute(reinterpret_cast<const void*>(&conv_bf16_ws16_kernel<false>), hipFuncAttributeMaxDynamicSharedMemorySize, W16_LDS_BYTES);
      if (e == hipSuccess)
        e = hipFuncSetAttribute(reinterpret_cast<const void*>(&conv_bf16_ws16_kernel<true>), hipFuncAttributeMaxDynamicSharedMemorySize, W16_LDS_BYTES);
      if (e != hipSuccess) {
        yogo_set_error("conv_bf16_ws16: hipFuncSetAttribute(MaxDynamicSharedMemorySize = %d) failed: %s", W16_LDS_BYTES, hipGetErrorString(e));
        return YOGO_ERR_HIP;
      }
      hipDeviceProp_t prop;
      n_cu_of[dev] = (hipGetDeviceProperties(&prop, dev) == hipSuccess && prop.multiProcessorCount > 0) ? prop.multiProcessorCount : 256;
    }
    n_cu = n_cu_of[dev];
  }
  if (p.ntiles <= 0) return YOGO_OK;
  if (p.act != ACT_NONE || p.signs != nullptr || p.chan_scale != nullptr || (p.nchunk & 3) != 0) {
    yogo_set_error("conv_bf16_ws16: plain epilogue and whole chunk-pair pairs only");
    return YOGO_ERR_ARG;
  }
  int grid = min(p.ntiles, n_cu);
  if (grid >= 8) grid &= ~7;
  if (p.bias != nullptr) hipLaunchKernelGGL(conv_bf16_ws16_kernel<true>, dim3(grid), dim3(512), W16_LDS_BYTES, stream, p);
  else hipLaunchKernelGGL(conv_bf16_ws16_kernel<false>, dim3(grid), dim3(512), W16_LDS_BYTES, stream, p);
  if (yogo_launch_log_enabled())
    yogo_launch_log("conv_bf16_ws16_kernel<%s> | Kb=%d in=%dx%d ncb=%d TW=%d tiles_per_band=%d periods=%d ntiles=%d grid=%d lds=%d", p.bias ? "true" : "false", p.Kb,
                    p.IH, p.IW, p.ncb, p.TW, p.tiles_per_band, 3 * (p.nchunk / 2), p.ntiles, grid, W16_LDS_BYTES);
  YOGO_CHECK_LAUNCH("conv_bf16_ws16");
  return YOGO_OK;
}
```

yogo_amd/engine.py:

```python
from __future__ import annotations

import threading
import weakref
from dataclasses import dataclass, field
from typing import Dict, List, Optional, Tuple

import torch
from torch import nn

from yogo_amd import _hip

ACT_NONE, ACT_LEAKY, ACT_SILU = 0, 1, 2


@dataclass
class Layer:
    conv: nn.Conv2d
    bn: Optional[nn.BatchNorm2d] = None
    act: int = ACT_NONE
    drop: Optional[nn.Dropout2d] = None

    @property
    def cin(self) -> int:
        return self.conv.in_channels
# ... 22 lines not shown
    z: Optional[torch.Tensor] = None
    pre: Optional[torch.Tensor] = None
    signs: Optional[torch.Tensor] = None
    signs0: Optional[torch.Tensor] = None
    w_used: Optional[torch.Tensor] = None
    gram: Optional[torch.Tensor] = None
    mask: Optional[torch.Tensor] = None
    mean: Optional[torch.Tensor] = None
    invstd: Optional[torch.Tensor] = None
    bn_train: bool = False


def parse_backbone(backbone: nn.Sequential) -> List[Layer]:
    layers: List[Layer] = []
    for blk in backbone:
        mods = [blk] if isinstance(blk, nn.Conv2d) else list(blk)
        if not mods or not isinstance(mods[0], nn.Conv2d):
            raise RuntimeError(f"yogo_amd: unsupported block {blk!r}: every block must start with nn.Conv2d")
        conv = mods[0]
        k, s, p = conv.kernel_size, conv.stride, conv.padding
        ok = k[0] == k[1] and s[0] == s[1] and conv.dilation == (1, 1) and conv.groups == 1 and conv.padding_mode == "zeros"
        ok = ok and ((k[0] == 3 and p == (1, 1) and s[0] in (1, 2)) or (k[0] == 1 and p == (0, 0) and s[0] == 1))
        if not ok:
            raise RuntimeError(f"yogo_amd: unsupported convolution {conv!r} (3x3 pad 1 stride 1|2, or 1x1)")
        L = Layer(conv=conv)
        for m in mods[1:]:
            if isinstance(m, nn.BatchNorm2d):
                L.bn = m
            elif isinstance(m, nn.LeakyReLU):
                if abs(m.negative_slope - 0.01) > 1e-12:
                    raise RuntimeError("yogo_amd: LeakyReLU slope must be 0.01")
                L.act = ACT_LEAKY
            elif isinstance(m, nn.SiLU):
                L.act = ACT_SILU
            elif isinstance(m, nn.Dropout2d):
                L.drop = m
            else:
                raise RuntimeError(f"yogo_amd: unsupported module {m!r} in block")
        if L.bn is not None and L.drop is not None:
            raise RuntimeError("yogo_amd: BatchNorm + Dropout2d in one block is not part of the block grammar")
        layers.append(L)
    return layers


def _f32(t: torch.Tensor) -> torch.Tensor:
    return t if (t.dtype == torch.float32 and t.is_contiguous()) else t.contiguous().float()


def _bn_affine(L: Layer, dev) -> Tuple[torch.Tensor, torch.Tensor]:
    bn = L.bn
    gamma = _f32(bn.weight.detach()) if bn.weight is not None else torch.ones(L.cout, device=dev)
    beta = _f32(bn.bias.detach()) if bn.bias is not None else torch.zeros(L.cout, device=dev)
    return gamma, beta


def _bn_grad_dst(bn: nn.BatchNorm2d, dst, grads: Dict[int, torch.Tensor], cout: int, dev) -> Tuple[torch.Tensor, torch.Tensor]:
    dgamma = dst(bn.weight) if bn.weight is not None else torch.empty(cout, dtype=torch.float32, device=dev)
    dbeta = dst(bn.bias) if bn.bias is not None else torch.empty(cout, dtype=torch.float32, device=dev)
    if bn.weight is not None:
        grads[id(bn.weight)] = dgamma
        grads[id(bn.bias)] = dbeta
    return dgamma, dbeta


def _bn_finalize(eng: "Engine", L: Layer, fn: str, *lead_args, count: int, dev, st) -> Tuple[torch.Tensor, torch.Tensor]:
    bn = L.bn
    mean = torch.empty(L.cout, dtype=torch.float32, device=dev)
    invstd = torch.empty(L.cout, dtype=torch.float32, device=dev)
    track = bn.track_running_stats and bn.running_mean is not None
    _hip.call(fn, *lead_args, L.cout, count, float(bn.eps), float(bn.momentum if bn.momentum is not None else 0.0), mean, invstd,
              bn.running_mean if track else None, bn.running_var if track else None, bn.num_batches_tracked if track else None, st)
    if track:
        eng.generation += 1
    return mean, invstd


def _pack_hit(eng: "Engine", key: Tuple[int, int], w: torch.Tensor) -> Optional[torch.Tensor]:
    hit = eng._pack.get(key)
    return hit[2] if hit is not None and hit[0] == w._version and hit[1] == w.data_ptr() else None


class Engine:
    def __init__(self, backbone: nn.Sequential):
        self.backbone_ref = weakref.ref(backbone)
        self.layers = parse_backbone(backbone)
        self._pack: Dict[Tuple[int, int], Tuple[int, int, torch.Tensor]] = {}
        self.clip: float = 0.0
        self.prof: Optional[list] = None
        self.prof_only: Optional[set] = None
        self._open = None
        self.generation: int = 0
        self._pack_multi = None
        self._drop_consts = None
        self._infer_bf16: Optional["InferEngineBF16"] = None

    def _tick(self, kind: str, layer: int, flops: float, mw: int = 0, nbytes: float = 0.0) -> None:
        if self.prof is not None and (self.prof_only is None or mw in self.prof_only):
            e0, e1 = torch.cuda.Event(enable_timing=True), torch.cuda.Event(enable_timing=True)
            e0.record()
            self._open = (kind, layer, mw, flops, e0, e1, nbytes)

    def _tock(self) -> None:
        if self._open is not None:
            self._open[5].record()
            self.prof.append(self._open)
            self._open = None

    def invalidate_packed(self) -> None:
        self._pack.clear()
        self.generation += 1

    def _packed(self, i: int, mode: int) -> torch.Tensor:
        L = self.layers[i]
        w = L.conv.weight
        key = (i, mode)
        buf = _pack_hit(self, key, w)
        if buf is not None:
            return buf
        nbytes = _hip.query_size("yogo_conv_packed_bytes", L.cin, L.cout, L.k, L.s, mode)
        buf = torch.empty(nbytes // 4, dtype=torch.float32, device=w.device)
        _hip.call("yogo_conv_pack_f32", _f32(w.detach()), buf, L.cin, L.cout, L.k, L.s, mode, _hip.stream_ptr())
        self._pack[key] = (w._version, w.data_ptr(), buf)
        return buf

    def _first_direct(self, i: int) -> bool:
        L = self.layers[i]
        return i == 0 and L.cin in (1, 3) and L.k == 3

    def forward(self, x: torch.Tensor, need_grad: bool) -> Tuple[torch.Tensor, List[Saved]]:
        _hip.require_cuda(x, "the input batch")
        if x.ndim != 4:
            raise RuntimeError(f"yogo_amd: expected a [B,C,H,W] batch, got {tuple(x.shape)}")
        dev = x.device
        st = _hip.stream_ptr()
        B = x.shape[0]
        if x.dtype == torch.uint8:
            cur = x.contiguous()
        else:
            cur = _f32(x)
        saved: List[Saved] = []
        for i, L in enumerate(self.layers):
            if cur.shape[1] != L.cin:
                raise RuntimeError(f"yogo_amd: layer {i} expects {L.cin} channels, got {cur.shape[1]}")
            IH, IW = int(cur.shape[2]), int(cur.shape[3])
            OH, OW = L.out_hw(IH, IW)
            if OH <= 0 or OW <= 0:
                raise RuntimeError(f"yogo_amd: image too small at layer {i}")
            w = L.conv.weight
            _hip.require_cuda(w, "the model parameters")
            bias = _f32(L.conv.bias.detach()) if L.conv.bias is not None else None
            S = Saved(x_in=cur)
            mask = None
            if L.drop is not None and L.drop.training and L.drop.p > 0:
                p = float(L.drop.p)
                mask = (torch.rand(B, L.cout, device=dev) >= p).to(torch.float32) / (1.0 - p)
                S.mask = mask
            has_bn = L.bn is not None
            bn_train = has_bn and (L.bn.training or L.bn.running_mean is None)
            out = torch.empty(B, L.cout, OH, OW, dtype=torch.float32, device=dev)
            pre = None
            if (not has_bn) and need_grad and L.act == ACT_SILU:
                pre = torch.empty_like(out)
            stats = None
            rows = mpad = 0
            direct = self._first_direct(i)
            if bn_train:
                if direct:
                    rows = _hip.query_ints("yogo_conv_first_stats_rows", 1, B, IH, IW, L.s)[0]
                    mpad = L.cout
                else:
                    rows, mpad = _hip.query_ints("yogo_conv2d_fwd_stats_shape", 2, B, L.cin, L.cout, IH, IW, L.k, L.s)
                stats = torch.empty(rows * mpad * 2, dtype=torch.float32, device=dev)
            fused_act = ACT_NONE if has_bn else L.act
            if direct:
                _hip.call("yogo_conv_first_fwd", cur, 0 if cur.dtype == torch.uint8 else 1, _f32(w.detach()), bias, out, pre,
                          mask, stats, B, L.cin, L.cout, IH, IW, L.s, fused_act, st)
            else:
                if cur.dtype != torch.float32:
                    cur = cur.float()
                    S.x_in = cur
                pk = self._packed(i, 0)
                self._tick("fwd", i, 2.0 * B * L.cout * L.cin * L.k * L.k * OH * OW, mw=4 if L.cout > 64 else (2 if L.cout > 32 else 1))
                _hip.call("yogo_conv2d_fwd_f32", cur, pk, bias, out, pre, mask, stats, B, L.cin, L.cout, IH, IW, L.k, L.s,
                          fused_act, st)
                self._tock()
            if has_bn:
                bn = L.bn
                gamma, beta = _bn_affine(L, dev)
                y = torch.empty_like(out) if need_grad else out
                if bn_train:
                    if bn.track_running_stats and bn.running_mean is not None and bn.momentum is None:
                        raise RuntimeError("yogo_amd: BatchNorm2d(momentum=None) is not supported")
                    mean, invstd = _bn_finalize(self, L, "yogo_bn_finalize", stats, rows, mpad, count=B * OH * OW, dev=dev, st=st)
                    _hip.call("yogo_bn_apply_act", out, y, mean, invstd, 0, float(bn.eps), gamma, beta, B, L.cout, OH * OW,
                              L.act, st)
                    S.mean, S.invstd = mean, invstd
                else:
                    _hip.call("yogo_bn_apply_act", out, y, bn.running_mean, bn.running_var, 1, float(bn.eps), gamma, beta, B,
                              L.cout, OH * OW, L.act, st)
                    if need_grad:
                        invstd = torch.empty(L.cout, dtype=torch.float32, device=dev)
                        _hip.call("yogo_bn_invstd", bn.running_var, float(bn.eps), invstd, L.cout, st)
                        S.mean, S.invstd = bn.running_mean, invstd
                S.bn_train = bn_train
                S.z = out if need_grad else None
                S.y = y
                cur = y
            else:
                S.y = out
                S.pre = pre
                cur = out
            saved.append(S if need_grad else Saved(x_in=cur))
        return cur, saved

    def backward(self, saved: List[Saved], graw: torch.Tensor,
                 grad_out: Optional[Dict[int, torch.Tensor]] = None, on_layer=None) -> List[Optional[torch.Tensor]]:
        st = _hip.stream_ptr()
        dev = graw.device
        clip = float(self.clip)
        grads: Dict[int, torch.Tensor] = {}

        def dst(param: torch.Tensor) -> torch.Tensor:
            if grad_out is not None and id(param) in grad_out:
                return grad_out[id(param)]
            return torch.empty(param.shape, dtype=torch.float32, device=dev)
        g = _f32(graw)
        n = len(self.layers)
        if g is graw and self.layers[-1].bn is not None:
            g = g.clone()
        for i in range(n - 1, -1, -1):
            L, S = self.layers[i], saved[i]
            B, _, OH, OW = g.shape
            IH, IW = int(S.x_in.shape[2]), int(S.x_in.shape[3])
            if L.bn is not None:
                bn = L.bn
                gamma, beta = _bn_affine(L, dev)
                dgamma, dbeta = _bn_grad_dst(bn, dst, grads, L.cout, dev)
                rows = _hip.query_ints("yogo_bn_bwd_rows", 1, B, OH * OW)[0]
                part = torch.empty(rows * L.cout * 2, dtype=torch.float32, device=dev)
                sums = torch.empty(2 * L.cout, dtype=torch.float32, device=dev)
                _hip.call("yogo_bn_bwd", g, S.z, g, S.mean, S.invstd, gamma, beta, L.act, dgamma, dbeta, part, sums, B, L.cout,
                          OH * OW, 1 if S.bn_train else 0, clip, st)
            dw = dst(L.conv.weight)
            has_bias = L.conv.bias is not None
            if self._first_direct(i):
                rows = _hip.query_ints("yogo_conv_first_wgrad_rows", 1, B, IH, IW, L.s)[0]
                nj = L.cin * 9 + 1
                part = torch.empty(rows * L.cout * nj, dtype=torch.float32, device=dev)
                x_in = S.x_in
                _hip.call("yogo_conv_first_wgrad", x_in, 0 if x_in.dtype == torch.uint8 else 1, g, part, B, L.cin, L.cout, IH,
                          IW, L.s, st)
                red = torch.empty(L.cout, nj, dtype=torch.float32, device=dev)
                _hip.call("yogo_partials_reduce", part, rows, L.cout * nj, clip, red, st)
                dw.copy_(red[:, : nj - 1].reshape(dw.shape))
                if has_bias:
                    db = dst(L.conv.bias)
                    db.copy_(red[:, nj - 1])
                    grads[id(L.conv.bias)] = db
            else:
                wsb = _hip.query_size("yogo_conv2d_wgrad_workspace_bytes", B, L.cin, L.cout, IH, IW, L.k, L.s)
                ws = torch.empty(wsb // 4, dtype=torch.float32, device=dev)
                db = dst(L.conv.bias) if has_bias else None
                self._tick("wgrad", i, 2.0 * B * L.cout * L.cin * L.k * L.k * OH * OW)
                _hip.call("yogo_conv2d_wgrad_f32", S.x_in, g, dw, db, ws, B, L.cin, L.cout, IH, IW, L.k, L.s, clip, st)
                self._tock()
                if has_bias:
                    grads[id(L.conv.bias)] = db
            grads[id(L.conv.weight)] = dw
            if on_layer is not None:
                on_layer(i)
            if i > 0:
                Lp, Sp = self.layers[i - 1], saved[i - 1]
                ref_act = Lp.act
                if Lp.bn is not None:
                    act_ref, ref_act = None, ACT_NONE
                elif Lp.act == ACT_SILU:
                    act_ref = Sp.pre
                    if act_ref is None:
                        raise RuntimeError("yogo_amd: missing saved pre-activation for a SiLU block")
                elif Lp.act == ACT_LEAKY:
                    act_ref = Sp.y
                else:
                    act_ref = None
                dx = torch.empty(B, L.cin, IH, IW, dtype=torch.float32, device=dev)
                pk = self._packed(i, 1)
                mw_tag = 20 if L.s == 2 else (4 if L.cin > 64 else (2 if L.cin > 32 else 1))
                self._tick("dgrad", i, 2.0 * B * L.cout * L.cin * L.k * L.k * OH * OW, mw=mw_tag)
                _hip.call("yogo_conv2d_dgrad_f32", g, pk, dx, act_ref, ref_act, Sp.mask, B, L.cin, L.cout, IH, IW, L.k, L.s, st)
                self._tock()
                g = dx
        bb = self.backbone_ref()
        return [grads.get(id(p)) for p in bb.parameters()]



def _blocks(c: int) -> int:
    return ((c + 15) // 16) * 2


_FUSE_LAYER0_BWD = True
_L0_NO_Z = True
_WGRAD_DEFER_REDUCE = True
_L01_FUSE_BWD = True
_HEAD_BN_FUSE = True


def _packed_bf16(eng: Engine, i: int, mode: int) -> torch.Tensor:
    L = eng.layers[i]
    w = L.conv.weight
    key = (i, 10 + mode)
    buf = _pack_hit(eng, key, w)
    if buf is not None:
        return buf
    nbytes = _hip.query_size("yogo_conv_bf16_packed_bytes", L.cin, L.cout, L.k, mode)
    buf = torch.empty(nbytes, dtype=torch.uint8, device=w.device)
    _hip.call("yogo_conv_bf16_pack", _f32(w.detach()), None, buf, L.cin, L.cout, L.k, mode, _hip.stream_ptr())
    eng._pack[key] = (w._version, w.data_ptr(), buf)
    return buf


def _pack_all_bf16(eng: Engine) -> None:
    jobs = [(i, mode) for i in range(1, len(eng.layers)) for mode in (0, 2 if (eng.layers[i].s == 2 and eng.layers[i].k == 3) else 1)]
    ws = [eng.layers[i].conv.weight for i, _ in jobs]
    if any(w.dtype != torch.float32 or not w.is_contiguous() for w in ws) or not jobs:
        return
    if all(_pack_hit(eng, (i, 10 + m), w) is not None for (i, m), w in zip(jobs, ws)):
        return
    dev = ws[0].device
    key = tuple(w.data_ptr() for w in ws)
    st = eng._pack_multi
    if st is None or st[0] != key:
        bufs, rows, blk = [], [], 0
        for (i, mode), w in zip(jobs, ws):
            L = eng.layers[i]
            buf = torch.empty(_hip.query_size("yogo_conv_bf16_packed_bytes", L.cin, L.cout, L.k, mode), dtype=torch.uint8, device=dev)
            bufs.append(buf)
            rows.append([w.data_ptr(), 0, buf.data_ptr(), L.cin, L.cout, L.k, mode, blk])
            blk += _hip.query_ints("yogo_conv_bf16_pack_blocks", 1, L.cin, L.cout, L.k, mode)[0]
        st = (key, bufs, torch.tensor(rows, dtype=torch.int64, device=dev), blk)
        eng._pack_multi = st
    _, bufs, table, blk = st
    _hip.call("yogo_conv_bf16_pack_multi", table, len(jobs), blk, _hip.stream_ptr())
    for (i, mode), w, buf in zip(jobs, ws, bufs):
        eng._pack[(i, 10 + mode)] = (w._version, w.data_ptr(), buf)


def _dropout_masks(eng: Engine, B: int, dev) -> Dict[int, torch.Tensor]:
    act = [(i, float(L.drop.p)) for i, L in enumerate(eng.layers) if L.drop is not None and L.drop.training and L.drop.p > 0]
    if not act:
        return {}
    key = (B, tuple(act), str(dev))
    cached = eng._drop_consts
    if cached is None or cached[0] != key:
        sizes = [B * eng.layers[i].cout for i, _ in act]
        pvec = torch.cat([torch.full((n,), p, dtype=torch.float32) for n, (_, p) in zip(sizes, act)]).to(dev)
        cached = (key, sizes, pvec, 1.0 / (1.0 - pvec))
        eng._drop_consts = cached
    _, sizes, pvec, inv_keep = cached
    m = (torch.rand(pvec.numel(), device=dev) >= pvec).to(torch.float32) * inv_keep
    out, off = {}, 0
    for n, (i, _) in zip(sizes, act):
        out[i] = m[off:off + n].view(B, eng.layers[i].cout)
        off += n
    return out


def _check_bf16_train_input(eng: Engine, x: torch.Tensor) -> None:
    _hip.require_cuda(x, "the input batch")
    if x.ndim != 4:
        raise RuntimeError(f"yogo_amd: expected a [B,C,H,W] batch, got {tuple(x.shape)}")
    if x.shape[1] != eng.layers[0].cin:
        raise RuntimeError(f"yogo_amd: layer 0 expects {eng.layers[0].cin} channels, got {x.shape[1]}")
    for j in range(1, len(eng.layers)):
        if eng.layers[j].cin != eng.layers[j - 1].cout:
            raise RuntimeError(f"yogo_amd: layer {j} expects {eng.layers[j].cin} channels, layer {j - 1} produces {eng.layers[j - 1].cout}")
    for Lj in eng.layers:
        bnj = Lj.bn
        if (bnj is not None and (bnj.training or bnj.running_mean is None) and bnj.track_running_stats
                and bnj.running_mean is not None and bnj.momentum is None):
            raise RuntimeError("yogo_amd: BatchNorm2d(momentum=None) is not supported")
    if not eng._first_direct(0):
        raise RuntimeError("yogo_amd: bf16 training needs a 1- or 3-channel 3x3 first convolution")


def _first_mfma_fwd_bf16(eng: Engine, L: Layer, S: Saved, bias, bn_train: bool, B: int, H: int, W: int, st) -> torch.Tensor:
    cur, dev = S.x_in, S.x_in.device
    OH, OW = L.out_hw(H, W)
    bn = L.bn
    gamma, beta = _bn_affine(L, dev)
    w32 = _f32(L.conv.weight.detach())
    y = torch.empty(B, _blocks(L.cout), OH, OW, 8, dtype=torch.bfloat16, device=dev)
    if bn_train:
        rows = _hip.query_ints("yogo_conv_first_gram_rows", 1, B, H, W)[0]
        gpart = torch.empty(rows * 54, dtype=torch.int32, device=dev)
        gram64 = torch.empty(90, dtype=torch.float64, device=dev)
        S.gram = torch.empty(90, dtype=torch.float32, device=dev)
        _hip.call("yogo_conv_first_gram", cur, gpart, gram64, S.gram, B, H, W, st)
        mean, invstd = _bn_finalize(eng, L, "yogo_bn_stats_from_gram", gram64, w32, bias, count=B * OH * OW, dev=dev, st=st)
    else:
        invstd = torch.empty(L.cout, dtype=torch.float32, device=dev)
        _hip.call("yogo_bn_invstd", bn.running_var, float(bn.eps), invstd, L.cout, st)
        mean = bn.running_mean
    no_z = (_L0_NO_Z and _FUSE_LAYER0_BWD and S.gram is not None and L.conv.bias is None
            and _hip.lib().yogo_conv_first_bn_wgrad_xs_supported(0, L.cin, L.cout, H, W, L.s, L.act))
    if no_z:
        out8 = None
        S.signs0 = torch.empty(B, OH * OW * 2, dtype=torch.uint8, device=dev)
        _hip.call("yogo_conv_first_mfma_signs", cur, w32, bias, None, y, S.signs0, mean, invstd, gamma, beta, B, L.cout, H, W, L.act, st)
    else:
        out8 = torch.empty_like(y)
        _hip.call("yogo_conv_first_mfma", cur, w32, bias, out8, y, mean, invstd, gamma, beta, None, B, L.cout, H, W, L.act, st)
    S.mean, S.invstd, S.bn_train, S.z, S.y = mean, invstd, bn_train, out8, y
    S.w_used = w32.to(torch.bfloat16).to(torch.float32)
    return y


def _layer_fwd_bf16(eng: Engine, i: int, L: Layer, S: Saved, bias, bn_train: bool, last: bool, B: int, H: int, W: int, st) -> torch.Tensor:
    cur, mask, dev = S.x_in, S.mask, S.x_in.device
    OH, OW = L.out_hw(H, W)
    has_bn = L.bn is not None
    if last and (has_bn or mask is not None):
        raise RuntimeError("yogo_amd: BatchNorm / Dropout on the last layer is not supported by the bf16 path")
    fused_act = ACT_NONE if has_bn else L.act
    out8 = None if last else torch.empty(B, _blocks(L.cout), OH, OW, 8, dtype=torch.bfloat16, device=dev)
    out32 = torch.empty(B, L.cout, OH, OW, dtype=torch.float32, device=dev) if last else None
    stats = None
    rows = mpad = 0
    if i == 0:
        if bn_train:
            rows, mpad = _hip.query_ints("yogo_conv_first_stats_rows", 1, B, H, W, L.s)[0], L.cout
            stats = torch.empty(rows * mpad * 2, dtype=torch.float32, device=dev)
        _hip.call("yogo_conv_first_fwd_train_bf16", cur, 0 if cur.dtype == torch.uint8 else 1, _f32(L.conv.weight.detach()), bias,
                  out8, mask, stats, B, L.cin, L.cout, H, W, L.s, fused_act, st)
    else:
        pk = _packed_bf16(eng, i, 0)
        nbytes = B * (_blocks(L.cin) * 8 * H * W * 2 + (L.cout * OH * OW * 4 if last else _blocks(L.cout) * 8 * OH * OW * 2))
        eng._tick("fwd", i, 2.0 * B * L.cout * L.cin * L.k * L.k * OH * OW, mw=34 if (L.cout > 64 and L.s == 1) else (35 if (L.cout > 64 and L.cin > 64 and L.k == 3) else 30), nbytes=nbytes)
        if L.act == ACT_SILU and not has_bn:
            S.pre = torch.empty_like(out8)
            _hip.call("yogo_conv2d_fwd_bf16_pre", cur, pk, bias, out8, S.pre, mask, B, L.cin, L.cout, H, W, L.k, L.s, fused_act, st)
        elif L.act == ACT_LEAKY and not has_bn and not last:
            S.signs = torch.empty(_hip.query_size("yogo_bf16_signs_bytes", B, L.cout, OH, OW), dtype=torch.uint8, device=dev)
            _hip.call("yogo_conv2d_fwd_bf16_signs", cur, pk, bias, out8, S.signs, mask, B, L.cin, L.cout, H, W, L.k, L.s, fused_act, st)
        else:
            _hip.call("yogo_conv2d_fwd_bf16", cur, pk, bias, out8, out32, mask, None, B, L.cin, L.cout, H, W, L.k, L.s, fused_act, st)
        eng._tock()
    if not has_bn:
        S.y = out32 if last else out8
        return S.y
    bn = L.bn
    gamma, beta = _bn_affine(L, dev)
    y = torch.empty_like(out8)
    if bn_train:
        if i > 0:
            rows, mpad = _hip.query_ints("yogo_bn_bwd_bf16_rows", 1, B, OH * OW)[0], L.cout
            stats = torch.empty(rows * mpad * 2, dtype=torch.float32, device=dev)
            _hip.call("yogo_bn_stats_bf16", out8, stats, B, L.cout, OH * OW, st)
        mean, invstd = _bn_finalize(eng, L, "yogo_bn_finalize", stats, rows, mpad, count=B * OH * OW, dev=dev, st=st)
    else:
        invstd = torch.empty(L.cout, dtype=torch.float32, device=dev)
        _hip.call("yogo_bn_invstd", bn.running_var, float(bn.eps), invstd, L.cout, st)
        mean = bn.running_mean
    _hip.call("yogo_bn_apply_act_bf16", out8, y, mean, invstd, 0, float(bn.eps), gamma, beta, B, L.cout, OH * OW, L.act, st)
    S.mean, S.invstd, S.bn_train, S.z, S.y = mean, invstd, bn_train, out8, y
    return y


def forward_bf16_train(eng: Engine, x: torch.Tensor) -> Tuple[torch.Tensor, List[Saved]]:
    _check_bf16_train_input(eng, x)
    dev, st, B = x.device, _hip.stream_ptr(), x.shape[0]
    _pack_all_bf16(eng)
    masks = _dropout_masks(eng, B, dev)
    cur = x.contiguous() if x.dtype == torch.uint8 else _f32(x)
    H, W = int(cur.shape[2]), int(cur.shape[3])
    saved: List[Saved] = []
    n = len(eng.layers)
    for i, L in enumerate(eng.layers):
        OH, OW = L.out_hw(H, W)
        if OH <= 0 or OW <= 0:
            raise RuntimeError(f"yogo_amd: image too small at layer {i}")
        last = i == n - 1
        has_bn = L.bn is not None
        if L.act == ACT_SILU and not has_bn and (i == 0 or last):
            raise RuntimeError("yogo_amd: bf16 training of a first / last SiLU block without BatchNorm is not implemented (use fp32)")
        bias = _f32(L.conv.bias.detach()) if L.conv.bias is not None else None
        S = Saved(x_in=cur, mask=masks.get(i))
        bn_train = has_bn and (L.bn.training or L.bn.running_mean is None)
        if (i == 0 and has_bn and S.mask is None and not last and cur.dtype == torch.uint8
                and _hip.lib().yogo_conv_first_mfma_supported(0, L.cin, L.cout, H, W, L.s)):
            cur = _first_mfma_fwd_bf16(eng, L, S, bias, bn_train, B, H, W, st)
        else:
            cur = _layer_fwd_bf16(eng, i, L, S, bias, bn_train, last, B, H, W, st)
        saved.append(S)
        H, W = OH, OW
    return cur, saved


def backward_bf16_train(eng: Engine, saved: List[Saved], graw: torch.Tensor,
                        grad_out: Optional[Dict[int, torch.Tensor]] = None, on_layer=None,
                        trace: Optional[dict] = None, flush_layers=None, stop_at: int = 0) -> List[Optional[torch.Tensor]]:
    n = len(eng.layers)
    if not 0 <= stop_at < n:
        raise ValueError(f"yogo_amd: stop_at {stop_at} is not a layer of this {n}-layer network")
    st, dev, clip = _hip.stream_ptr(), graw.device, float(eng.clip)
    grads: Dict[int, torch.Tensor] = {}

    def dst(param: torch.Tensor) -> torch.Tensor:
        if grad_out is not None and id(param) in grad_out:
            return grad_out[id(param)]
        return torch.empty(param.shape, dtype=torch.float32, device=dev)

    queued_ws: List[torch.Tensor] = []
    wq = _wgrad_queue() if (_WGRAD_DEFER_REDUCE and (on_layer is None or flush_layers is not None)) else None
    flush_at = frozenset(flush_layers) if flush_layers is not None else frozenset()
    if wq is not None:
        _hip.call("yogo_wgrad_reduce_queue_reset", wq)
    if graw.dtype == torch.bfloat16 and graw.ndim == 5:
        g = graw
        B = g.shape[0]
    else:
        graw = _f32(graw)
        B, P, Sy, Sx = graw.shape
        g = torch.empty(B, _blocks(P), Sy, Sx, 8, dtype=torch.bfloat16, device=dev)
        _hip.call("yogo_nchw_f32_to_bf16_8c", graw, g, B, P, Sy * Sx, st)

    def bn_backward(L, S, g, head_g, OH, OW):
        gamma, beta = _bn_affine(L, dev)
        dgamma, dbeta = _bn_grad_dst(L.bn, dst, grads, L.cout, dev)
        rows = _hip.query_ints("yogo_bn_bwd_bf16_rows", 1, B, OH * OW)[0]
        part = torch.empty(rows * L.cout * 2, dtype=torch.float32, device=dev)
        sums = torch.empty(2 * L.cout, dtype=torch.float32, device=dev)
        if head_g is not None:
            dz = torch.empty(B, _blocks(L.cout), OH, OW, 8, dtype=torch.bfloat16, device=dev)
            _hip.call("yogo_bn_bwd_bf16_head", *head_g, S.z, dz, S.mean, S.invstd, gamma, beta, L.act, dgamma, dbeta,
                      part, sums, B, L.cout, OH * OW, 1 if S.bn_train else 0, clip, st)
        else:
            dz = g
            _hip.call("yogo_bn_bwd_bf16", g, S.z, dz, S.mean, S.invstd, gamma, beta, L.act, dgamma, dbeta, part, sums, B, L.cout, OH * OW,
                      1 if S.bn_train else 0, clip, st)
        return dz

    def wgrad_first_bn(L, S, g, fused01, dw, IH, IW):
        gamma, beta = _bn_affine(L, dev)
        dgamma, dbeta = _bn_grad_dst(L.bn, dst, grads, L.cout, dev)
        cols = _hip.query_ints("yogo_conv_first_bn_wgrad_cols", 1, L.cin, L.cout)[0]
        sums = torch.empty(cols, dtype=torch.float32, device=dev)
        xg = "_xs" if S.signs0 is not None else "_xg" if S.gram is not None else ""
        if fused01 is not None:
            part, rows = fused01[:2]
        else:
            rows = _hip.query_ints("yogo_conv_first_wgrad_rows", 1, B, IH, IW, L.s)[0]
            part = torch.empty(rows * cols, dtype=torch.float32, device=dev)
            _hip.call("yogo_conv_first_bn_wgrad_bf16" + xg, S.x_in, 0 if S.x_in.dtype == torch.uint8 else 1, g,
                      S.signs0 if S.signs0 is not None else S.z, S.mean, S.invstd, gamma, beta, part, B, L.cin, L.cout, IH, IW, L.s, L.act, st)
        _hip.call("yogo_partials_reduce", part, rows, cols, 0.0, sums, st)
        _hip.call("yogo_conv_first_bn_wgrad_finalize" + xg, sums, *((S.gram,) if S.gram is not None else ()), S.mean, S.invstd, gamma,
                  S.w_used if S.w_used is not None else _f32(L.conv.weight.detach()), dw, dgamma,
                  dbeta, B, L.cin, L.cout, IH, IW, L.s, 1 if S.bn_train else 0, clip, st)

    def wgrad_dgrad_first(L, S, g, dw, db, IH, IW, OH, OW):
        L0, S0 = eng.layers[0], saved[0]
        ws = torch.empty(_hip.query_size("yogo_conv2d_dgrad_wgrad_first_bwd_workspace_bytes", B, IH, IW) // 4, dtype=torch.float32, device=dev)
        rows = _hip.query_ints("yogo_conv2d_dgrad_first_bwd_rows", 1, B, IH, IW, 1)[0]
        cols = _hip.query_ints("yogo_conv_first_bn_wgrad_cols", 1, L0.cin, L0.cout)[0]
        part = torch.empty(rows * cols, dtype=torch.float32, device=dev)
        queued_ws.append(ws)
        eng._tick("wgrad", 1, 2.0 * B * L.cout * L.cin * L.k * L.k * OH * OW * 2, mw=30,
                  nbytes=B * (16 * (_blocks(L.cout) + _blocks(L.cin)) * OH * OW + 2 * IH * IW + 4 * IH * IW))
        _hip.call("yogo_conv2d_dgrad_wgrad_bf16_first_bwd", g, _packed_bf16(eng, 1, 1), S.x_in, S0.x_in, S0.signs0, part, dw, db, ws,
                  B, L.cin, L.cout, IH, IW, L0.act, clip, wq, st)
        eng._tock()
        return part, rows, IH, IW

    def wgrad_first(L, S, g, dw, db, IH, IW):
        rows = _hip.query_ints("yogo_conv_first_wgrad_rows", 1, B, IH, IW, L.s)[0]
        nj = L.cin * 9 + 1
        part = torch.empty(rows * L.cout * nj, dtype=torch.float32, device=dev)
        red = torch.empty(L.cout, nj, dtype=torch.float32, device=dev)
        _hip.call("yogo_conv_first_wgrad_bf16g", S.x_in, 0 if S.x_in.dtype == torch.uint8 else 1, g, part, B, L.cin, L.cout, IH, IW, L.s, st)
        _hip.call("yogo_partials_reduce", part, rows, L.cout * nj, clip, red, st)
        dw.view(L.cout, nj - 1).copy_(red[:, : nj - 1])
        if db is not None:
            db.copy_(red[:, nj - 1])

    def wgrad(i, L, S, g, dw, db, IH, IW, OH, OW):
        ws = torch.empty(_hip.query_size("yogo_conv2d_wgrad_bf16_workspace_bytes", B, L.cin, L.cout, IH, IW, L.k, L.s) // 4,
                         dtype=torch.float32, device=dev)
        eng._tick("wgrad", i, 2.0 * B * L.cout * L.cin * L.k * L.k * OH * OW, mw=30,
                  nbytes=B * 2 * 8 * (_blocks(L.cout) * OH * OW + _blocks(L.cin) * IH * IW))
        if wq is not None:
            queued_ws.append(ws)
            _hip.call("yogo_conv2d_wgrad_bf16_deferred", S.x_in, g, dw, db, ws, B, L.cin, L.cout, IH, IW, L.k, L.s, clip, wq, st)
        else:
            _hip.call("yogo_conv2d_wgrad_bf16", S.x_in, g, dw, db, ws, B, L.cin, L.cout, IH, IW, L.k, L.s, clip, st)
        eng._tock()

    def dgrad(i, L, g, Sp, act_ref, ref_act, IH, IW, OH, OW):
        pk = _packed_bf16(eng, i, 2 if (L.s == 2 and L.k == 3) else 1)
        dx = torch.empty(B, _blocks(L.cin), IH, IW, 8, dtype=torch.bfloat16, device=dev)
        signs = Sp.signs if ref_act == ACT_LEAKY else None
        if signs is not None:
            nbytes = B * (16 * _blocks(L.cout) * OH * OW + 17 * _blocks(L.cin) * IH * IW)
        else:
            nbytes = B * 2 * 8 * (_blocks(L.cout) * OH * OW + _blocks(L.cin) * IH * IW * (2 if act_ref is not None else 1))
        eng._tick("dgrad", i, 2.0 * B * L.cout * L.cin * L.k * L.k * OH * OW, mw=34 if (L.cin > 64 and L.s == 1 and act_ref is None) else 30, nbytes=nbytes)
        if signs is not None:
            _hip.call("yogo_conv2d_dgrad_bf16_signs", g, pk, dx, signs, Sp.mask, B, L.cin, L.cout, IH, IW, L.k, L.s, st)
        else:
            _hip.call("yogo_conv2d_dgrad_bf16", g, pk, dx, act_ref, ref_act, Sp.mask, B, L.cin, L.cout, IH, IW, L.k, L.s, st)
        eng._tock()
        return dx

    head_g = None
    fused01 = None
    for i in range(n - 1, stop_at - 1, -1):
        L, S = eng.layers[i], saved[i]
        OH, OW = (int(g.shape[2]), int(g.shape[3])) if g is not None else fused01[2:]
        IH, IW = int(S.x_in.shape[2]), int(S.x_in.shape[3])
        Lp, Sp = (eng.layers[i - 1], saved[i - 1]) if i > stop_at else (None, None)
        fuse0 = _FUSE_LAYER0_BWD and i == 0 and L.bn is not None and L.conv.bias is None and L.act in (ACT_NONE, ACT_LEAKY)
        fuse01 = False
        if _L01_FUSE_BWD and i == 1 and stop_at == 0 and _FUSE_LAYER0_BWD:
            fuse01 = bool(Sp.signs0 is not None and Sp.x_in.dtype == torch.uint8 and Lp.bn is not None and Lp.conv.bias is None and Lp.cin == 1
                          and Lp.s == 2 and Lp.act in (ACT_NONE, ACT_LEAKY) and L.k == 3 and L.s == 1 and Sp.mask is None
                          and _hip.lib().yogo_conv2d_dgrad_first_bwd_supported(L.cin, L.cout, IH, IW, B, Lp.act))
        head_below = bool(_HEAD_BN_FUSE and i == n - 1 and Lp is not None and i - 1 > 0 and L.k == 1 and L.s == 1 and L.cout <= 16
                          and Lp.bn is not None and Lp.cout % 16 == 0 and g.shape[1] == 2)
        act_ref, ref_act = None, ACT_NONE
        if Lp is not None and Lp.bn is None and Lp.act != ACT_NONE:
            act_ref, ref_act = (Sp.y if Lp.act == ACT_LEAKY else Sp.pre), Lp.act
        if trace is not None and g is not None and head_g is None:
            trace[("g", i)] = g.clone()
        if L.bn is not None and not fuse0:
            g, head_g = bn_backward(L, S, g, head_g, OH, OW), None
            if trace is not None:
                trace[("dz", i)] = g.clone()
        dw = dst(L.conv.weight)
        db = dst(L.conv.bias) if L.conv.bias is not None else None
        if fuse0:
            wgrad_first_bn(L, S, g, fused01, dw, IH, IW)
        elif fuse01:
            fused01 = wgrad_dgrad_first(L, S, g, dw, db, IH, IW, OH, OW)
        elif i == 0:
            wgrad_first(L, S, g, dw, db, IH, IW)
        else:
            wgrad(i, L, S, g, dw, db, IH, IW, OH, OW)
        if db is not None:
            grads[id(L.conv.bias)] = db
        grads[id(L.conv.weight)] = dw
        if on_layer is not None:
            if wq is not None and i in flush_at:
                _hip.call("yogo_wgrad_reduce_flush", wq, st)
            on_layer(i)
        if fuse01:
            g = None
        elif head_below:
            head_g = (g, _f32(L.conv.weight.detach()).reshape(L.cout, L.cin), L.cout)
        elif i > stop_at:
            g = dgrad(i, L, g, Sp, act_ref, ref_act, IH, IW, OH, OW)
    if wq is not None:
        _hip.call("yogo_wgrad_reduce_flush", wq, st)
    bb = eng.backbone_ref()
    return [grads.get(id(p)) for p in bb.parameters()]


_WGRAD_QUEUE = None


def _wgrad_queue() -> int:
    global _WGRAD_QUEUE
    if _WGRAD_QUEUE is None:
        import ctypes
        h = ctypes.c_void_p(0)
        _hip.call("yogo_wgrad_reduce_queue_create", ctypes.addressof(h))
        _WGRAD_QUEUE = int(h.value)
    return _WGRAD_QUEUE


_ENGINES: "weakref.WeakKeyDictionary[nn.Module, Engine]" = weakref.WeakKeyDictionary()


def get_engine(backbone: nn.Sequential) -> Engine:
    eng = _ENGINES.get(backbone)
    if eng is None:
        eng = Engine(backbone)
        _ENGINES[backbone] = eng
    return eng


class _BackboneFn(torch.autograd.Function):
    @staticmethod
    def forward(ctx, x, backbone, *params):
        eng = get_engine(backbone)
        raw, saved = eng.forward(x, need_grad=True)
        ctx.eng = eng
        ctx.saved = saved
        return raw

    @staticmethod
    def backward(ctx, graw):
        with torch.cuda.device(graw.device):
            grads = ctx.eng.backward(ctx.saved, graw)
        ctx.saved = None
        return (None, None, *grads)


_BF16_BWD_LOCK = threading.Lock()


def bf16_training_requested() -> bool:
    return bf16_inference_requested()


def bf16_train_supported(eng: Engine) -> bool:
    layers = eng.layers
    n = len(layers)
    if n < 2 or not eng._first_direct(0):
        return False
    for i, L in enumerate(layers):
        if i > 0 and L.cin != layers[i - 1].cout:
            return False
        if L.act == ACT_SILU and L.bn is None and i in (0, n - 1):
            return False
        if L.bn is not None and L.bn.momentum is None:
            return False
    return layers[-1].bn is None and layers[-1].drop is None


def _param_layers(eng: Engine) -> Dict[int, int]:
    out: Dict[int, int] = {}
    for i, L in enumerate(eng.layers):
        for m in (L.conv, L.bn):
            if m is not None:
                for p in m.parameters(recurse=False):
                    out[id(p)] = i
    return out


def bf16_autograd_backward(eng: Engine, saved: List[Saved], g: torch.Tensor, needs) -> List[Optional[torch.Tensor]]:
    bb = eng.backbone_ref()
    params = list(bb.parameters())
    needs = list(needs)
    if len(needs) != len(params):
        raise RuntimeError("yogo_amd: the backbone's parameters changed between forward and backward")
    if not any(needs):
        return [None] * len(params)
    layer_of = _param_layers(eng)
    lo = min(layer_of[id(p)] for p, nd in zip(params, needs) if nd)
    with _BF16_BWD_LOCK:
        grads = backward_bf16_train(eng, saved, g, stop_at=lo if lo >= 2 else 0)
    return [gr if nd else None for gr, nd in zip(grads, needs)]


class _BackboneBF16Fn(torch.autograd.Function):

    @staticmethod
    def forward(ctx, x, backbone, *params):
        eng = get_engine(backbone)
        with torch.cuda.device(x.device):
            raw, saved = forward_bf16_train(eng, x)
        ctx.save_for_backward(*params)
        ctx.eng, ctx.saved = eng, saved
        return raw

    @staticmethod
    def backward(ctx, graw):
        if ctx.saved is None:
            raise RuntimeError("yogo_amd: a second backward through a bf16 training graph is not supported (its forward records "
                               "belong to the first backward); run the forward again")
        ctx.saved_tensors
        saved, ctx.saved = ctx.saved, None
        with torch.cuda.device(graw.device):
            grads = bf16_autograd_backward(ctx.eng, saved, graw, ctx.needs_input_grad[2:])
        return (None, None, *grads)


def backbone_apply(backbone: nn.Sequential, x: torch.Tensor) -> torch.Tensor:
    _hip.require_cuda(x, "the input batch")
    params = list(backbone.parameters())
    if not backbone.training and not torch.is_grad_enabled() and (
            bf16_inference_requested() or getattr(backbone, "bf16_inference", False)):
        raw = backbone_infer_bf16(backbone, x)
        if raw is not None:
            return raw
    with torch.cuda.device(x.device):
        if torch.is_grad_enabled() and any(p.requires_grad for p in params):
            if bf16_training_requested() and bf16_train_supported(get_engine(backbone)):
                return _BackboneBF16Fn.apply(x, backbone, *params)
            return _BackboneFn.apply(x, backbone, *params)
        raw, _ = get_engine(backbone).forward(x, need_grad=False)
        return raw

class InferEngineBF16:

    def __init__(self, engine: Engine):
        self.engine = engine
        self._key = None
        self._prep: List[Tuple[Optional[torch.Tensor], Optional[torch.Tensor]]] = []

    def _state_key(self):
        k = [self.engine.generation]
        for L in self.engine.layers:
            ts = [L.conv.weight, L.conv.bias]
            if L.bn is not None:
                ts += [L.bn.weight, L.bn.bias, L.bn.running_mean, L.bn.running_var]
            for t in ts:
                k.append(None if t is None else (t.data_ptr(), t._version))
        return tuple(k)

    def supported(self) -> bool:
        L0 = self.engine.layers[0]
        if not (L0.cin in (1, 3) and L0.k == 3):
            return False
        return all(L.bn is None or (not L.bn.training and L.bn.running_mean is not None) for L in self.engine.layers)

    @torch.no_grad()
    def _prepare(self) -> None:
        key = self._state_key()
        if key == self._key:
            return
        st = _hip.stream_ptr()
        prep = []
        for i, L in enumerate(self.engine.layers):
            w = _f32(L.conv.weight.detach())
            bias = L.conv.bias.detach().float() if L.conv.bias is not None else None
            scale = None
            if L.bn is not None:
                bn = L.bn
                gamma = bn.weight.detach().float() if bn.weight is not None else torch.ones_like(bn.running_var)
                beta = bn.bias.detach().float() if bn.bias is not None else torch.zeros_like(bn.running_var)
                scale = gamma / torch.sqrt(bn.running_var.float() + bn.eps)
                base = bias if bias is not None else torch.zeros_like(scale)
                bias = beta + (base - bn.running_mean.float()) * scale
            if i == 0:
                wf = w * scale[:, None, None, None] if scale is not None else w
                prep.append((wf.contiguous(), bias.contiguous() if bias is not None else None))
            else:
                nbytes = _hip.query_size("yogo_conv_bf16_packed_bytes", L.cin, L.cout, L.k, 0)
                packed = torch.empty(nbytes, dtype=torch.uint8, device=w.device)
                _hip.call("yogo_conv_bf16_pack", w, scale.contiguous() if scale is not None else None, packed, L.cin, L.cout, L.k, 0, st)
                prep.append((packed, bias.contiguous() if bias is not None else None))
        self._prep = prep
        self._key = key

    @torch.no_grad()
    def forward(self, x: torch.Tensor, decode=None) -> torch.Tensor:
        _hip.require_cuda(x, "the input batch")
        if x.ndim != 4:
            raise RuntimeError(f"yogo_amd: expected a [B,C,H,W] batch, got {tuple(x.shape)}")
        self._prepare()
        st = _hip.stream_ptr()
        dev = x.device
        B = x.shape[0]
        cur = x.contiguous() if x.dtype == torch.uint8 else _f32(x)
        H, W = int(cur.shape[2]), int(cur.shape[3])
        n = len(self.engine.layers)
        for i, L in enumerate(self.engine.layers):
            OH, OW = L.out_hw(H, W)
            if OH <= 0 or OW <= 0:
                raise RuntimeError(f"yogo_amd: image too small at layer {i}")
            wq, bias = self._prep[i]
            last = i == n - 1
            if i == 0:
                if cur.shape[1] != L.cin:
                    raise RuntimeError(f"yogo_amd: layer 0 expects {L.cin} channels, got {cur.shape[1]}")
                mb = _hip.lib().yogo_bf16_channel_blocks(L.cout)
                out = torch.empty(B, mb, OH, OW, 8, dtype=torch.bfloat16, device=dev)
                if cur.dtype == torch.uint8 and _hip.lib().yogo_conv_first_mfma_supported(0, L.cin, L.cout, H, W, L.s):
                    _hip.call("yogo_conv_first_mfma", cur, wq, bias, out, None, None, None, None, None, None, B, L.cout, H, W, L.act, st)
                else:
                    _hip.call("yogo_conv_first_fwd_bf16", cur, 0 if cur.dtype == torch.uint8 else 1, wq, bias, out, B, L.cin, L.cout, H, W,
                              L.s, L.act, st)
                if last:
                    raise RuntimeError("yogo_amd: a one-layer network is not supported by the bf16 inference path")
            elif last:
                out = torch.empty(B, L.cout, OH, OW, dtype=torch.float32, device=dev)
                if decode is not None and head_decode_fusable(L):
                    cxs, cys, aw, ah, wm, hm, inference = decode
                    cxs, cys = _hip.grid_buffers(cxs, cys, OH, OW, dev)
                    _hip.call("yogo_head1x1_decode_fwd_bf16", cur, wq, bias, out, cxs, cys, B, L.cin, L.cout, OH, OW, aw, ah, wm, hm, 1 if inference else 0, st)
                    self.decoded = True
                else:
                    _hip.call("yogo_conv2d_fwd_bf16", cur, wq, bias, None, out, None, None, B, L.cin, L.cout, H, W, L.k, L.s, L.act, st)
                    self.decoded = False
            else:
                mb = _hip.lib().yogo_bf16_channel_blocks(L.cout)
                out = torch.empty(B, mb, OH, OW, 8, dtype=torch.bfloat16, device=dev)
                _hip.call("yogo_conv2d_fwd_bf16", cur, wq, bias, out, None, None, None, B, L.cin, L.cout, H, W, L.k, L.s, L.act, st)
            cur, H, W = out, OH, OW
        return cur


def head_decode_fusable(L) -> bool:
    return L.k == 1 and L.s == 1 and L.bn is None and L.act == 0 and 6 <= L.cout <= 16 and L.cin % 16 == 0 and L.cin <= 128


def bf16_inference_requested() -> bool:
    try:
        return bool(torch.is_autocast_enabled()) and torch.get_autocast_gpu_dtype() == torch.bfloat16
    except Exception:
        return False


def backbone_infer_bf16(backbone: nn.Sequential, x: torch.Tensor, decode=None):
    eng = get_engine(backbone)
    inf = eng._infer_bf16
    if inf is None:
        inf = eng._infer_bf16 = InferEngineBF16(eng)
    if not inf.supported():
        return None
    with torch.cuda.device(x.device):
        if decode is None:
            return inf.forward(x)
        out = inf.forward(x, decode=decode)
        return out, bool(inf.decoded)
```

Baseline: 11000 images/s.

## Fuse BatchNorm backward reduction into dgrad conv epilogue for 128-channel layers

Adds a BN-reduction mode to the warp-specialized bf16 dgrad conv kernel. While storing dx it re-reads the matching pre-BN activations z via LDS DMA and accumulates per-channel sum(g·act') and sum(g·act'·xhat) with DPP butterflies into per-block partials. The following BN backward then skips its separate reduce pass over g and z and runs only finalize and apply. This saves one full read of two activation tensors per eligible layer, at the cost of extra LDS, a serialized drain phase in the epilogue, and more kernel complexity.

After: 10870 images/s. -1.2%, worse.

```diff
diff --git a/include/yogo_hip.h b/include/yogo_hip.h
--- a/include/yogo_hip.h
+++ b/include/yogo_hip.h
@@ -159,6 +159,14 @@
 int yogo_bn_bwd_bf16_head(const void* gh, const float* head_w, int P, const void* z, void* dz, const float* mean, const float* invstd,
                           const float* gamma, const float* beta, int act, float* dgamma, float* dbeta, float* part, float* sums, int B,
                           int C, int HW, int training, float clip, yogo_stream_t stream);
+int yogo_conv2d_dgrad_bf16_bnred_supported(int B, int Cin, int Cout, int IH, int IW, int ksize, int stride, int act);
+int yogo_conv2d_dgrad_bf16_bnred_rows(int B, int Cin, int Cout, int IH, int IW, int ksize, int stride, int* rows);
+int yogo_conv2d_dgrad_bf16_bnred(const void* dy, const void* packed_dgrad, void* dx, const void* z, const float* mean, const float* invstd,
+                                 const float* gamma, const float* beta, int act, float* part, int B, int Cin, int Cout, int IH, int IW,
+                                 int ksize, int stride, yogo_stream_t stream);
+int yogo_bn_bwd_bf16_from_part(const void* g, const void* z, void* dz, const float* mean, const float* invstd, const float* gamma,
+                               const float* beta, int act, float* dgamma, float* dbeta, const float* part, int rows, float* sums, int B,
+                               int C, int HW, int training, float clip, yogo_stream_t stream);
 int yogo_nchw_f32_to_bf16_8c(const float* in, void* out, int B, int C, int HW, yogo_stream_t stream);
 int yogo_bf16_8c_to_nchw_f32(const void* in, float* out, int B, int C, int HW, yogo_stream_t stream);
 
diff --git a/yogo_amd/csrc/bn.hip b/yogo_amd/csrc/bn.hip
--- a/yogo_amd/csrc/bn.hip
+++ b/yogo_amd/csrc/bn.hip
@@ -537,6 +537,22 @@
   return YOGO_OK;
 }
 
+extern "C" int yogo_bn_bwd_bf16_from_part(const void* g, const void* z, void* dz, const float* mean, const float* invstd, const float* gamma,
+                                          const float* beta, int act, float* dgamma, float* dbeta, const float* part, int rows, float* sums, int B,
+                                          int C, int HW, int training, float clip, hipStream_t stream) {
+  YOGO_CHECK_ARG(g && z && dz && mean && invstd && gamma && beta && dgamma && dbeta && part && sums, "bn_bwd_bf16_from_part: null pointer");
+  YOGO_CHECK_ARG(B > 0 && C > 0 && HW > 0 && rows > 0, "bn_bwd_bf16_from_part: bad shape");
+  const int Cb = cb_of(C), nb = plane_blocks(HW, 4);
+  YOGO_CHECK_ARG(B * Cb <= 65535, "bn_bwd_bf16_from_part: batch * channel blocks exceeds 65535");
+  const u32x4_t* g4 = reinterpret_cast<const u32x4_t*>(g);
+  const u32x4_t* z4 = reinterpret_cast<const u32x4_t*>(z);
+  hipLaunchKernelGGL(bn_bwd_finalize_kernel, dim3(C), dim3(256), 0, stream, part, rows, C, clip, dgamma, dbeta, sums, sums + C);
+  hipLaunchKernelGGL(bn_bwd_apply_8c_kernel, dim3(nb, B * Cb), dim3(256), 0, stream, g4, z4, reinterpret_cast<u32x4_t*>(dz), mean,
+                     invstd, gamma, beta, act, sums, sums + C, 1.0f / ((float)B * (float)HW), training, C, Cb, HW);
+  YOGO_CHECK_LAUNCH("bn_bwd_bf16_from_part");
+  return YOGO_OK;
+}
+
 typedef float f32x4_t __attribute__((ext_vector_type(4)));
 typedef unsigned int u32x2_t __attribute__((ext_vector_type(2)));
 typedef __bf16 bf16x4_t __attribute__((ext_vector_type(4)));
diff --git a/yogo_amd/csrc/conv_bf16.hip b/yogo_amd/csrc/conv_bf16.hip
--- a/yogo_amd/csrc/conv_bf16.hip
+++ b/yogo_amd/csrc/conv_bf16.hip
@@ -1506,6 +1506,41 @@
                           IH, IW, ks, 1, (stride == 2 && ks == 3) ? 1 : 0, ACT_NONE, stream, nullptr, nullptr);
 }
 
+static bool bf_bnred_plan(ConvWsParams* q, int B, int Cin, int Cout, int IH, int IW, int ks, int stride) {
+  if (!g_bf_ws || g_bf_ws16 == 0 || ks != 3 || stride != 1 || Cin != 128 || B <= 0) return false;
+  *q = ConvWsParams{};
+  q->B = B; q->Kb = bf_kb_of(Cout); q->IH = IH; q->IW = IW; q->act = ACT_NONE;
+  if (!conv_bf16_ws_eligible(Cout, Cin, IH, IW, B) || !conv_bf16_ws16_eligible(Cout, Cin, IH, IW, B) || !conv_bf16_ws_plan(q)) return false;
+  return q->nchunk >= 8;
+}
+extern "C" int yogo_conv2d_dgrad_bf16_bnred_supported(int B, int Cin, int Cout, int IH, int IW, int ks, int stride, int act) {
+  ConvWsParams q;
+  if (act != ACT_NONE && act != ACT_LEAKY) return 0;
+  if (B <= 0 || Cin <= 0 || Cout <= 0 || IH <= 0 || IW <= 0) return 0;
+  return bf_bnred_plan(&q, B, Cin, Cout, IH, IW, ks, stride) ? 1 : 0;
+}
+extern "C" int yogo_conv2d_dgrad_bf16_bnred_rows(int B, int Cin, int Cout, int IH, int IW, int ks, int stride, int* rows) {
+  YOGO_CHECK_ARG(rows != nullptr, "conv2d_dgrad_bf16_bnred_rows: null");
+  ConvWsParams q;
+  YOGO_CHECK_ARG(bf_bnred_plan(&q, B, Cin, Cout, IH, IW, ks, stride), "conv2d_dgrad_bf16_bnred_rows: unsupported shape");
+  const int r = conv_bf16_ws16_bn_rows(q);
+  if (r < 0) return YOGO_ERR_HIP;
+  *rows = r;
+  return YOGO_OK;
+}
+extern "C" int yogo_conv2d_dgrad_bf16_bnred(const void* dy, const void* packed_dgrad, void* dx, const void* z, const float* mean, const float* invstd,
+                                            const float* gamma, const float* beta, int act, float* part, int B, int Cin, int Cout, int IH, int IW, int ks,
+                                            int stride, hipStream_t stream) {
+  YOGO_CHECK_ARG(dy && packed_dgrad && dx && z && mean && invstd && gamma && beta && part, "conv2d_dgrad_bf16_bnred: null pointer");
+  YOGO_CHECK_ARG(act == ACT_NONE || act == ACT_LEAKY, "conv2d_dgrad_bf16_bnred: ACT_NONE / ACT_LEAKY only");
+  if (int e = check_bf16_conv(B, Cin, Cout, IH, IW, ks, stride)) return e;
+  ConvWsParams q;
+  YOGO_CHECK_ARG(bf_bnred_plan(&q, B, Cin, Cout, IH, IW, ks, stride), "conv2d_dgrad_bf16_bnred: unsupported shape (ask yogo_conv2d_dgrad_bf16_bnred_supported)");
+  q.in = dy; q.wp = packed_dgrad; q.out = dx;
+  q.bn_z = z; q.bn_mean = mean; q.bn_invstd = invstd; q.bn_gamma = gamma; q.bn_beta = beta; q.bn_part = part; q.bn_act = act;
+  return launch_conv_bf16_ws16(q, stream);
+}
+
 extern "C" int yogo_conv_first_fwd_bf16(const void* in, int in_dtype, const float* w, const float* bias, void* out, int B,
                                         int Cin, int Cout, int IH, int IW, int stride, int act, hipStream_t stream) {
   YOGO_CHECK_ARG(in && w && out, "conv_first_fwd_bf16: null pointer");
diff --git a/yogo_amd/csrc/conv_bf16_ws.h b/yogo_amd/csrc/conv_bf16_ws.h
--- a/yogo_amd/csrc/conv_bf16_ws.h
+++ b/yogo_amd/csrc/conv_bf16_ws.h
@@ -25,6 +25,10 @@
   int ncb, TW, tiles_per_band, gx, ntiles;
   unsigned m_gx, m_tpb, m_bw, m_bwl, m_lw, m_lwl;
   int nchunk, act;
+  const void* bn_z;
+  const float *bn_mean, *bn_invstd, *bn_gamma, *bn_beta;
+  float* bn_part;
+  int bn_act;
 #ifdef YOGO_DIAG
   int dbg;
   unsigned long long* stamps;
diff --git a/yogo_amd/csrc/conv_bf16_ws16.h b/yogo_amd/csrc/conv_bf16_ws16.h
--- a/yogo_amd/csrc/conv_bf16_ws16.h
+++ b/yogo_amd/csrc/conv_bf16_ws16.h
@@ -9,7 +9,11 @@
 #define W16_EB (W16_STG + 32768)
 #define W16_MB (W16_EB + 512)
 #define W16_MBS (W16_MB + 1024)
-#define W16_LDS_BYTES (W16_MBS + 16)
+#define W16_BNC (W16_MBS + 16)
+#define W16_BN (W16_BNC + 2048)
+#define W16_BZ (W16_BN + 4096)
+#define W16_LDS_BYTES (W16_BZ + 8192)
 
 bool conv_bf16_ws16_eligible(int K, int M, int IH, int IW, int B);
 int launch_conv_bf16_ws16(const ConvWsParams& p, hipStream_t stream);
+int conv_bf16_ws16_bn_rows(const ConvWsParams& p);
diff --git a/yogo_amd/csrc/conv_bf16_ws16.hip b/yogo_amd/csrc/conv_bf16_ws16.hip
--- a/yogo_amd/csrc/conv_bf16_ws16.hip
+++ b/yogo_amd/csrc/conv_bf16_ws16.hip
@@ -49,6 +49,21 @@
                : "memory", "scc");
 #undef W16_PJ
 #undef W16_PK
+}
+__device__ __forceinline__ void w16_dma2(i32x4 rs, unsigned lds, int voff, unsigned so0, unsigned so1) {
+  asm volatile(
+      "s_mov_b32 m0, %2\n\ts_nop 4\n\tbuffer_load_dwordx4 %0, %1, %3 offen lds\n\t"
+      "s_add_u32 m0, m0, 1024\n\ts_nop 0\n\tbuffer_load_dwordx4 %0, %1, %4 offen lds"
+      ::"v"(voff), "s"(rs), "s"(lds), "s"(so0), "s"(so1) : "memory", "scc");
+}
+__device__ __forceinline__ u32x4 w16_dead() {
+  u32x4 d;
+  asm volatile("" : "=v"(d));
+  return d;
+}
+__device__ __forceinline__ u32x4 w16_opaque(u32x4 v) {
+  asm("" : "+v"(v));
+  return v;
 }
 __device__ __forceinline__ void w16_store16(u32x4 data, int voff, i32x4 rs, unsigned soff) {
   asm volatile("s_nop 4\n\tbuffer_store_dwordx4 %0, %1, %2, %3 offen" ::"v"(data), "v"(voff), "s"(rs), "s"(soff) : "memory");
@@ -112,9 +127,22 @@
 
   unsigned k_ord = 0;
   TileS T{};
-  if (!find_tile(k_ord, T)) return;
+  const bool bnred = p.bn_part != nullptr;
+  if (!find_tile(k_ord, T)) {
+    if (bnred) {
+      p.bn_part[(size_t)blockIdx.x * 1024 + tid] = 0.f;
+      p.bn_part[(size_t)blockIdx.x * 1024 + 512 + tid] = 0.f;
+    }
+    return;
+  }
 
   if (tid < 128) ldsf[W16_EB / 4 + tid] = (BIAS && p.bias != nullptr) ? p.bias[tid] : 0.f;
+  if (bnred && tid < 128) {
+    ldsf[W16_BNC / 4 + tid * 4 + 0] = p.bn_mean[tid];
+    ldsf[W16_BNC / 4 + tid * 4 + 1] = p.bn_invstd[tid];
+    ldsf[W16_BNC / 4 + tid * 4 + 2] = p.bn_gamma[tid];
+    ldsf[W16_BNC / 4 + tid * 4 + 3] = p.bn_beta[tid];
+  }
   __syncthreads();
 
   if (team == 1) {
@@ -163,26 +191,9 @@
     auto req_i = [&](i32x4 rs, const int (&voff)[WS_NI], int cn, int ps, int j) {
       w16_dma4(rs, (unsigned)(W16_I0 + ps * W16_ISLOT + j * WS_IB + tw * 64 * 16), voff[0], voff[1], voff[2], voff[3], (unsigned)cn * so_i);
     };
-    const unsigned stg_rd = (unsigned)(W16_STG + tw * 8192 + lane * 16);
-    u32x4 fifo[8];
-    int f_vo = (int)OOB;
-    i32x4 f_rs = w16_rsrc(p.out, 0u);
-    int f_cb0 = 0;
-    auto fifo_fill = [&](int cb0, int vop, i32x4 rs_o) {
-#pragma unroll
-      for (int u = 0; u < 8; ++u) fifo[u] = *reinterpret_cast<const u32x4*>(lds + stg_rd + u * 1024);
-      f_vo = vop; f_rs = rs_o; f_cb0 = cb0;
-    };
-    auto fifo_store4 = [&](auto h_tag) {
-      constexpr int Hh = decltype(h_tag)::value;
-      const i32x4 rs = {__builtin_amdgcn_readfirstlane(f_rs.x), __builtin_amdgcn_readfirstlane(f_rs.y), __builtin_amdgcn_readfirstlane(f_rs.z),
-                        __builtin_amdgcn_readfirstlane(f_rs.w)};
-      const int cb0 = __builtin_amdgcn_readfirstlane(f_cb0);
-#pragma unroll
-      for (int u = 4 * Hh; u < 4 * Hh + 4; ++u) w16_store16(fifo[u], (W16_ABL & 2) ? (int)OOB : f_vo, rs, (unsigned)(cb0 + u) * (unsigned)plane16);
-    };
     using IC0 = std::integral_constant<int, 0>;
     using IC1 = std::integral_constant<int, 1>;
+
 
     int voff[WS_NI];
     decode_slots(T, voff);
@@ -197,20 +208,114 @@
     req_w(0, 0, 0);
     asm volatile("s_waitcnt vmcnt(0)" ::: "memory");
     __builtin_amdgcn_s_barrier();
-    bool has_next = true;
-    TileS Tn{};
-    int voff_n[WS_NI] = {(int)OOB, (int)OOB, (int)OOB, (int)OOB}, vo_n = (int)OOB;
-    i32x4 rs_in_n = rs_in, rs_out_n = rs_out;
-    while (has_next) {
+    auto run = [&](auto bn_tag) {
+      constexpr bool BN = decltype(bn_tag)::value;
+      const float bn_slope = p.bn_act == ACT_LEAKY ? LEAKY_SLOPE : 1.f;
+      typedef float f32x2 __attribute__((ext_vector_type(2)));
+      typedef float f32x4 __attribute__((ext_vector_type(4)));
+      f32x2* const bn_acc = reinterpret_cast<f32x2*>(lds + W16_BN) + tw * 128 + (lane & 15);
+      if (BN && lane < 16) {
+#pragma unroll
+        for (int a = 0; a < 8; ++a) bn_acc[a * 16] = f32x2{0.f, 0.f};
+      }
+#define W16_BFLY(A, B, BIT, CTRL) \
+    (((BIT) ? (B) : (A)) + __builtin_bit_cast(float, __builtin_amdgcn_update_dpp(0, __builtin_bit_cast(int, (BIT) ? (A) : (B)), CTRL, 0xf, 0xf, false)))
+      auto bn_term = [&](unsigned gw, unsigned zw, int j, unsigned cst_at, float& ge, float& gx) {
+        const f32x4 cst = *reinterpret_cast<const f32x4*>(lds + cst_at);
+        const float gf = __builtin_bit_cast(float, (j & 1) ? (gw & 0xFFFF0000u) : (gw << 16));
+        const float zf = __builtin_bit_cast(float, (j & 1) ? (zw & 0xFFFF0000u) : (zw << 16));
+        const float xh = (zf - cst.x) * cst.y;
+        ge = gf * (fmaf(xh, cst.z, cst.w) > 0.f ? 1.f : bn_slope);
+        gx = ge * xh;
+      };
+      auto bn_unit = [&](u32x4 g4, u32x4 z4, int cb, bool valid, float& rg, float& rx) {
+        float wg[4], wx[4];
+        const unsigned cst0 = (unsigned)W16_BNC + (unsigned)cb * 128u;
+#pragma unroll
+        for (int j = 0; j < 4; ++j) {
+          float ge0, gx0, ge1, gx1;
+          bn_term(valid ? g4[j >> 1] : 0u, z4[j >> 1], j, cst0 + j * 16, ge0, gx0);
+          bn_term(valid ? g4[2 + (j >> 1)] : 0u, z4[2 + (j >> 1)], j, cst0 + (j + 4) * 16, ge1, gx1);
+          wg[j] = W16_BFLY(ge0, ge1, (lane & 8) != 0, 0x140);
+          wx[j] = W16_BFLY(gx0, gx1, (lane & 8) != 0, 0x140);
+          __builtin_amdgcn_sched_barrier(0);
+        }
+        const float xg0 = W16_BFLY(wg[0], wg[2], (lane & 4) != 0, 0x141), xg1 = W16_BFLY(wg[1], wg[3], (lane & 4) != 0, 0x141);
+        const float xx0 = W16_BFLY(wx[0], wx[2], (lane & 4) != 0, 0x141), xx1 = W16_BFLY(wx[1], wx[3], (lane & 4) != 0, 0x141);
+        rg = W16_BFLY(xg0, xg1, (lane & 2) != 0, 0x4E);
+        rx = W16_BFLY(xx0, xx1, (lane & 2) != 0, 0x4E);
+      };
+
+      const unsigned stg_rd = (unsigned)(W16_STG + tw * 8192 + lane * 16);
+      u32x4 fifo[8];
+      int f_vo = (int)OOB;
+      i32x4 f_rs = w16_rsrc(p.out, 0u);
+      int f_cb0 = 0;
+      auto fifo_fill = [&](int cb0, int vop, i32x4 rs_o) {
+#pragma unroll
+        for (int u = 0; u < 8; ++u) fifo[u] = *reinterpret_cast<const u32x4*>(lds + stg_rd + u * 1024);
+        f_vo = vop; f_rs = rs_o; f_cb0 = cb0;
+      };
+      auto fifo_store4 = [&](auto h_tag) {
+        constexpr int Hh = decltype(h_tag)::value;
+        const i32x4 rs = {__builtin_amdgcn_readfirstlane(f_rs.x), __builtin_amdgcn_readfirstlane(f_rs.y), __builtin_amdgcn_readfirstlane(f_rs.z),
+                          __builtin_amdgcn_readfirstlane(f_rs.w)};
+        const int cb0 = __builtin_amdgcn_readfirstlane(f_cb0);
+#pragma unroll
+        for (int u = 4 * Hh; u < 4 * Hh + 4; ++u) w16_store16(fifo[u], (W16_ABL & 2) ? (int)OOB : f_vo, rs, (unsigned)(cb0 + u) * (unsigned)plane16);
+      };
+      const unsigned bz = (unsigned)(W16_BZ + tw * 2048);
+      auto bn_zreq = [&](int s) {
+        unsigned long long a = ((unsigned long long)(unsigned)__builtin_amdgcn_readfirstlane(f_rs.x) |
+                                ((unsigned long long)((unsigned)__builtin_amdgcn_readfirstlane(f_rs.y) & 0xFFFFu) << 32)) +
+                               (unsigned long long)(reinterpret_cast<const unsigned char*>(p.bn_z) - reinterpret_cast<const unsigned char*>(p.out));
+        const i32x4 rs = {(int)(unsigned)a, (int)((unsigned)(a >> 32) & 0xFFFFu), __builtin_amdgcn_readfirstlane(f_rs.z), __builtin_amdgcn_readfirstlane(f_rs.w)};
+        const unsigned so = (unsigned)(2 * s) * (unsigned)plane16;
+        w16_dma2(rs, bz, f_vo, so, so + (unsigned)plane16);
+      };
+
+      auto bn_step = [&](int s) {
+        const u32x4 za = *reinterpret_cast<const u32x4*>(lds + bz + lane * 16), zb = *reinterpret_cast<const u32x4*>(lds + bz + 1024 + lane * 16);
+        const int k = s & 3;
+        const bool valid = f_vo != (int)OOB;
+        const int cb = 2 * s;
+        float ag, ax, bg, bx;
+        u32x4 gu;
+  #define W16_PICK(U) gu = w16_opaque(fifo[U]);
+        if (k == 0) W16_PICK(0) else if (k == 1) W16_PICK(2) else if (k == 2) W16_PICK(4) else W16_PICK(6)
+        bn_unit(gu, za, cb, valid, ag, ax);
+        __builtin_amdgcn_sched_barrier(0);
+        if (k == 0) W16_PICK(1) else if (k == 1) W16_PICK(3) else if (k == 2) W16_PICK(5) else W16_PICK(7)
+  #undef W16_PICK
+        bn_unit(gu, zb, cb + 1, valid, bg, bx);
+        float rg = W16_BFLY(ag, bg, (lane & 1) != 0, 0xB1), rx = W16_BFLY(ax, bx, (lane & 1) != 0, 0xB1);
+        rg += __shfl_xor(rg, 16, 64);
+        rx += __shfl_xor(rx, 16, 64);
+        rg += __shfl_xor(rg, 32, 64);
+        rx += __shfl_xor(rx, 32, 64);
+        if (lane < 16) {
+          f32x2 v = bn_acc[s * 16];
+          v.x += rg;
+          v.y += rx;
+          bn_acc[s * 16] = v;
+        }
+      };
+      bool has_next = true;
+      TileS Tn{};
+      int voff_n[WS_NI] = {(int)OOB, (int)OOB, (int)OOB, (int)OOB}, vo_n = (int)OOB;
+      i32x4 rs_in_n = rs_in, rs_out_n = rs_out;
       int P = 0, r = 0;
-      for (int c = 0; c < nper; ++c) {
+      auto period = [&](auto ph_tag, int c) {
+        constexpr int PH = decltype(ph_tag)::value;
+        constexpr int SC = PH == 0 ? 0 : PH == 2 ? 4 : (PH >= 10 && PH <= 13) ? PH - 10 : -1;
+        auto at = [&](int c0) { return SC == c0; };
         {
           const int rn = r == 2 ? 0 : r + 1, Pn = r == 2 ? P + 1 : P;
           if ((W16_ABL & 1) && c >= 1) {
           } else if (c + 1 < nper) req_w(Pn, rn, (c + 1) & 1);
           else if (has_next) req_w(0, 0, 0);
         }
-        if (c == 0) {
+        if (at(0)) {
           fifo_fill(0, vo_prev, rs_out_prev);
           asm volatile("s_waitcnt lgkmcnt(0)" ::: "memory");
           if (!(W16_ABL & 4)) __builtin_amdgcn_s_barrier();
@@ -230,12 +335,19 @@
             req = true;
           }
         }
-        if (c == 0) fifo_store4(IC0{});
+        if (PH >= 1 && PH <= 3) {
+          if (req) asm volatile("s_waitcnt vmcnt(10)" ::: "memory");
+          else asm volatile("s_waitcnt vmcnt(6)" ::: "memory");
+          bn_step(c - 1);
+        }
+        constexpr int c8 = BN ? 4 : 2;
+        if (at(0)) fifo_store4(IC0{});
         else if (c == 1) fifo_store4(IC1{});
-        else if (c == 2) { fifo_fill(8, vo_prev, rs_out_prev); fifo_store4(IC0{}); }
-        else if (c == 3) fifo_store4(IC1{});
-        const bool dr = c < 4;
-        if (c == 0) {
+        else if (at(c8)) { fifo_fill(8, vo_prev, rs_out_prev); fifo_store4(IC0{}); }
+        else if (c == c8 + 1) fifo_store4(IC1{});
+        const bool dr = c < 2 || c == c8 || c == c8 + 1;
+        const bool zr = BN && c < 8;
+        if (at(0)) {
           unsigned kn = k_ord + 1;
           has_next = find_tile(kn, Tn);
           k_ord = kn;
@@ -252,28 +364,71 @@
           if (tw == 0 && lane == 0) *reinterpret_cast<u32x4*>(lds + W16_MBS) = u32x4{has_next ? 1u : 0u, lw16_, perkb16_, 0u};
           asm volatile("s_waitcnt lgkmcnt(0)" ::: "memory");
         }
-        if (dr && req) asm volatile("s_waitcnt vmcnt(8)" ::: "memory");
+        if (zr) bn_zreq(c);
+        if (zr) {
+          if (dr && req) asm volatile("s_waitcnt vmcnt(10)" ::: "memory");
+          else if (dr || req) asm volatile("s_waitcnt vmcnt(6)" ::: "memory");
+          else asm volatile("s_waitcnt vmcnt(2)" ::: "memory");
+        } else if (dr && req) asm volatile("s_waitcnt vmcnt(8)" ::: "memory");
         else if (dr || req) asm volatile("s_waitcnt vmcnt(4)" ::: "memory");
         else asm volatile("s_waitcnt vmcnt(0)" ::: "memory");
         __builtin_amdgcn_s_barrier();
         if (++r == 3) { r = 0; ++P; }
+      };
+      while (has_next) {
+        P = 0; r = 0;
+#pragma unroll
+        for (int u = 0; u < 8; ++u) fifo[u] = w16_dead();
+        if constexpr (BN) {
+          period(std::integral_constant<int, 0>{}, 0);
+          for (int c = 1; c < 4; ++c) period(std::integral_constant<int, 1>{}, c);
+          period(std::integral_constant<int, 2>{}, 4);
+          for (int c = 5; c < 9; ++c) period(std::integral_constant<int, 3>{}, c);
+          for (int c = 9; c < nper; ++c) period(std::integral_constant<int, 4>{}, c);
+        } else {
+          period(std::integral_constant<int, 10>{}, 0);
+          period(std::integral_constant<int, 11>{}, 1);
+          period(std::integral_constant<int, 12>{}, 2);
+          period(std::integral_constant<int, 13>{}, 3);
+          for (int c = 4; c < nper; ++c) period(std::integral_constant<int, 14>{}, c);
+        }
+        vo_prev = vo;
+        rs_out_prev = rs_out;
+        if (has_next) {
+          vo = vo_n;
+          rs_out = rs_out_n;
+        }
       }
-      vo_prev = vo;
-      rs_out_prev = rs_out;
-      if (has_next) {
-        vo = vo_n;
-        rs_out = rs_out_n;
+      fifo_fill(0, vo_prev, rs_out_prev);
+      asm volatile("s_waitcnt lgkmcnt(0)" ::: "memory");
+      if (!(W16_ABL & 4)) __builtin_amdgcn_s_barrier();
+      fifo_store4(IC0{});
+      fifo_store4(IC1{});
+      auto bn_drain = [&](int h) {
+        for (int s = 4 * h; s < 4 * h + 4; ++s) {
+          bn_zreq(s);
+          asm volatile("s_waitcnt vmcnt(0)" ::: "memory");
+          bn_step(s);
+        }
+      };
+      if constexpr (BN) bn_drain(0);
+      __builtin_amdgcn_s_barrier();
+      fifo_fill(8, vo_prev, rs_out_prev);
+      fifo_store4(IC0{});
+      fifo_store4(IC1{});
+      if constexpr (BN) {
+        bn_drain(1);
+        if (lane < 16) {
+          float* row = p.bn_part + ((size_t)blockIdx.x * 4 + tw) * 256;
+          const int chl = (lane & 1) * 8 + ((lane >> 3) & 1) * 4 + ((lane >> 2) & 1) * 2 + ((lane >> 1) & 1);
+#pragma unroll
+          for (int a = 0; a < 8; ++a) *reinterpret_cast<f32x2*>(row + (a * 16 + chl) * 2) = bn_acc[a * 16];
+        }
       }
-    }
-    fifo_fill(0, vo_prev, rs_out_prev);
-    asm volatile("s_waitcnt lgkmcnt(0)" ::: "memory");
-    if (!(W16_ABL & 4)) __builtin_amdgcn_s_barrier();
-    fifo_store4(IC0{});
-    fifo_store4(IC1{});
-    __builtin_amdgcn_s_barrier();
-    fifo_fill(8, vo_prev, rs_out_prev);
-    fifo_store4(IC0{});
-    fifo_store4(IC1{});
+    };
+#undef W16_BFLY
+    if (bnred) run(std::true_type{});
+    else run(std::false_type{});
     return;
   }
 
@@ -316,13 +471,14 @@
   return Kb >= 8 && (Kb % 8) == 0;
 }
 
-int launch_conv_bf16_ws16(const ConvWsParams& p, hipStream_t stream) {
+namespace {
+int w16_grid(int ntiles) {
   static std::mutex mu;
   static int n_cu_of[64] = {0};
   int dev = 0;
   if (hipGetDevice(&dev) != hipSuccess || dev < 0 || dev >= 64) {
     yogo_set_error("conv_bf16_ws16: hipGetDevice failed");
-    return YOGO_ERR_HIP;
+    return -1;
   }
   int n_cu;
   {
@@ -333,24 +489,42 @@
         e = hipFuncSetAttribute(reinterpret_cast<const void*>(&conv_bf16_ws16_kernel<true>), hipFuncAttributeMaxDynamicSharedMemorySize, W16_LDS_BYTES);
       if (e != hipSuccess) {
         yogo_set_error("conv_bf16_ws16: hipFuncSetAttribute(MaxDynamicSharedMemorySize = %d) failed: %s", W16_LDS_BYTES, hipGetErrorString(e));
-        return YOGO_ERR_HIP;
+        return -1;
       }
       hipDeviceProp_t prop;
       n_cu_of[dev] = (hipGetDeviceProperties(&prop, dev) == hipSuccess && prop.multiProcessorCount > 0) ? prop.multiProcessorCount : 256;
     }
     n_cu = n_cu_of[dev];
   }
+  int grid = min(max(ntiles, 0), n_cu);
+  if (grid >= 8) grid &= ~7;
+  return grid;
+}
+}
+
+int conv_bf16_ws16_bn_rows(const ConvWsParams& p) {
+  const int grid = w16_grid(p.ntiles);
+  return grid < 0 ? -1 : 4 * grid;
+}
+
+int launch_conv_bf16_ws16(const ConvWsParams& p, hipStream_t stream) {
+  const int grid = w16_grid(p.ntiles);
+  if (grid < 0) return YOGO_ERR_HIP;
   if (p.ntiles <= 0) return YOGO_OK;
   if (p.act != ACT_NONE || p.signs != nullptr || p.chan_scale != nullptr || (p.nchunk & 3) != 0) {
     yogo_set_error("conv_bf16_ws16: plain epilogue and whole chunk-pair pairs only");
     return YOGO_ERR_ARG;
   }
-  int grid = min(p.ntiles, n_cu);
-  if (grid >= 8) grid &= ~7;
+  const bool bnred = p.bn_part != nullptr;
+  if (bnred && (p.bias != nullptr || p.nchunk < 8 || !p.bn_z || !p.bn_mean || !p.bn_invstd || !p.bn_gamma || !p.bn_beta ||
+                (p.bn_act != ACT_NONE && p.bn_act != ACT_LEAKY))) {
+    yogo_set_error("conv_bf16_ws16: the BatchNorm reduction needs no bias, >= 128 input channels, every BatchNorm tensor and ACT_NONE / ACT_LEAKY");
+    return YOGO_ERR_ARG;
+  }
   if (p.bias != nullptr) hipLaunchKernelGGL(conv_bf16_ws16_kernel<true>, dim3(grid), dim3(512), W16_LDS_BYTES, stream, p);
   else hipLaunchKernelGGL(conv_bf16_ws16_kernel<false>, dim3(grid), dim3(512), W16_LDS_BYTES, stream, p);
   if (yogo_launch_log_enabled())
-    yogo_launch_log("conv_bf16_ws16_kernel<%s> | Kb=%d in=%dx%d ncb=%d TW=%d tiles_per_band=%d periods=%d ntiles=%d grid=%d lds=%d", p.bias ? "true" : "false", p.Kb,
+    yogo_launch_log("conv_bf16_ws16_kernel<%s> | %sKb=%d in=%dx%d ncb=%d TW=%d tiles_per_band=%d periods=%d ntiles=%d grid=%d lds=%d", p.bias ? "true" : "false", bnred ? "bnred=1 " : "", p.Kb,
                     p.IH, p.IW, p.ncb, p.TW, p.tiles_per_band, 3 * (p.nchunk / 2), p.ntiles, grid, W16_LDS_BYTES);
   YOGO_CHECK_LAUNCH("conv_bf16_ws16");
   return YOGO_OK;
diff --git a/yogo_amd/engine.py b/yogo_amd/engine.py
--- a/yogo_amd/engine.py
+++ b/yogo_amd/engine.py
@@ -348,6 +348,7 @@
 _L0_NO_Z = True
 _WGRAD_DEFER_REDUCE = True
 _L01_FUSE_BWD = True
+_BN_REDUCE_IN_DGRAD = True
 _HEAD_BN_FUSE = True
 
 
@@ -570,9 +571,14 @@
         g = torch.empty(B, _blocks(P), Sy, Sx, 8, dtype=torch.bfloat16, device=dev)
         _hip.call("yogo_nchw_f32_to_bf16_8c", graw, g, B, P, Sy * Sx, st)
 
-    def bn_backward(L, S, g, head_g, OH, OW):
+    def bn_backward(L, S, g, head_g, OH, OW, given=None):
         gamma, beta = _bn_affine(L, dev)
         dgamma, dbeta = _bn_grad_dst(L.bn, dst, grads, L.cout, dev)
+        if given is not None:
+            sums = torch.empty(2 * L.cout, dtype=torch.float32, device=dev)
+            _hip.call("yogo_bn_bwd_bf16_from_part", g, S.z, g, S.mean, S.invstd, gamma, beta, L.act, dgamma, dbeta, given[0], given[1], sums,
+                      B, L.cout, OH * OW, 1 if S.bn_train else 0, clip, st)
+            return g
         rows = _hip.query_ints("yogo_bn_bwd_bf16_rows", 1, B, OH * OW)[0]
         part = torch.empty(rows * L.cout * 2, dtype=torch.float32, device=dev)
         sums = torch.empty(2 * L.cout, dtype=torch.float32, device=dev)
@@ -641,6 +647,19 @@
             _hip.call("yogo_conv2d_wgrad_bf16", S.x_in, g, dw, db, ws, B, L.cin, L.cout, IH, IW, L.k, L.s, clip, st)
         eng._tock()
 
+    def dgrad_bnred(i, L, g, Lp, Sp, IH, IW, OH, OW):
+        pk = _packed_bf16(eng, i, 1)
+        dx = torch.empty(B, _blocks(L.cin), IH, IW, 8, dtype=torch.bfloat16, device=dev)
+        rows = _hip.query_ints("yogo_conv2d_dgrad_bf16_bnred_rows", 1, B, L.cin, L.cout, IH, IW, L.k, L.s)[0]
+        part = torch.empty(rows * L.cin * 2, dtype=torch.float32, device=dev)
+        gamma, beta = _bn_affine(Lp, dev)
+        eng._tick("dgrad", i, 2.0 * B * L.cout * L.cin * L.k * L.k * OH * OW, mw=34,
+                  nbytes=B * 2 * 8 * (_blocks(L.cout) * OH * OW + 2 * _blocks(L.cin) * IH * IW))
+        _hip.call("yogo_conv2d_dgrad_bf16_bnred", g, pk, dx, Sp.z, Sp.mean, Sp.invstd, gamma, beta, Lp.act, part, B, L.cin, L.cout, IH, IW,
+                  L.k, L.s, st)
+        eng._tock()
+        return dx, (part, rows)
+
     def dgrad(i, L, g, Sp, act_ref, ref_act, IH, IW, OH, OW):
         pk = _packed_bf16(eng, i, 2 if (L.s == 2 and L.k == 3) else 1)
         dx = torch.empty(B, _blocks(L.cin), IH, IW, 8, dtype=torch.bfloat16, device=dev)
@@ -659,6 +678,7 @@
 
     head_g = None
     fused01 = None
+    bn_given = None
     for i in range(n - 1, stop_at - 1, -1):
         L, S = eng.layers[i], saved[i]
         OH, OW = (int(g.shape[2]), int(g.shape[3])) if g is not None else fused01[2:]
@@ -678,9 +698,10 @@
         if trace is not None and g is not None and head_g is None:
             trace[("g", i)] = g.clone()
         if L.bn is not None and not fuse0:
-            g, head_g = bn_backward(L, S, g, head_g, OH, OW), None
+            g, head_g = bn_backward(L, S, g, head_g, OH, OW, bn_given), None
             if trace is not None:
                 trace[("dz", i)] = g.clone()
+        bn_given = None
         dw = dst(L.conv.weight)
         db = dst(L.conv.bias) if L.conv.bias is not None else None
         if fuse0:
@@ -703,7 +724,11 @@
         elif head_below:
             head_g = (g, _f32(L.conv.weight.detach()).reshape(L.cout, L.cin), L.cout)
         elif i > stop_at:
-            g = dgrad(i, L, g, Sp, act_ref, ref_act, IH, IW, OH, OW)
+            if (_BN_REDUCE_IN_DGRAD and i - 1 > 0 and Lp.bn is not None and act_ref is None and Sp.mask is None and Lp.act in (ACT_NONE, ACT_LEAKY)
+                    and Sp.z is not None and _hip.lib().yogo_conv2d_dgrad_bf16_bnred_supported(B, L.cin, L.cout, IH, IW, L.k, L.s, Lp.act)):
+                g, bn_given = dgrad_bnred(i, L, g, Lp, Sp, IH, IW, OH, OW)
+            else:
+                g = dgrad(i, L, g, Sp, act_ref, ref_act, IH, IW, OH, OW)
     if wq is not None:
         _hip.call("yogo_wgrad_reduce_flush", wq, st)
     bb = eng.backbone_ref()
```
